# uw-x/AcousticSwarms-Speech

Measured on AMD Instinct MI355X. Metric: TDoA candidates/sec (shift+normalise+spot forward+energies), higher is better.
Workload: dtype f32 via f16x3 split-operand MFMA (fp32 accumulate); 1 GPU; configs[2] scene: 5-speaker reverberant mixture (image sources), 7 mics, T=48000 samples (BASELINE's '3 s @ 16 kHz' sample count; the reference pipeline and this scene generator run at 48 kHz, where it is a 1 s clip -- the reference-native 3 s is extras.T144000), fine-stage (Strict=1) candidate batch of one mixture, FULL spot net 47.27 M params, seeded random weights; internal_batch=256, parallelism=candidate-shard x1

## Files before the change

### acousticswarms-speech_amd/csrc/model_common.h

```cpp
#pragma once
#include <cstdlib>
#include <iterator>
#include <map>
#include <memory>
#include <string>
#include <vector>

#include "asw_common.h"

namespace asw_model {

struct DevBuf {
  float* p = nullptr;
  size_t n = 0;
  DevBuf() = default;
  DevBuf(const DevBuf&) = delete;
  DevBuf& operator=(const DevBuf&) = delete;
  DevBuf(DevBuf&& o) noexcept : p(o.p), n(o.n) { o.p = nullptr; o.n = 0; }
  ~DevBuf() { if (p) (void)hipFree(p); }
  int upload(const std::vector<float>& h) {
    if (p) { (void)hipFree(p); p = nullptr; }
    n = h.size();
    if (hipMalloc(&p, n * sizeof(float)) != hipSuccess) return asw::set_error(ASW_ERR_NOMEM, "hipMalloc(%zu floats)", n);
    ASW_HIP(hipMemcpy(p, h.data(), n * sizeof(float), hipMemcpyHostToDevice));
    return ASW_OK;
  }
};

struct WBuf {
  DevBuf f32;
  uint16_t* hi = nullptr;
  uint16_t* lo = nullptr;
  int32_t shift = 0;
  WBuf() = default;
  WBuf(const WBuf&) = delete;
  WBuf& operator=(const WBuf&) = delete;
  WBuf(WBuf&& o) noexcept : f32(std::move(o.f32)), hi(o.hi), lo(o.lo), shift(o.shift), fhi(o.fhi), flo(o.flo) {
    o.hi = o.lo = o.fhi = o.flo = nullptr;
  }
  ~WBuf() {
    if (hi) (void)hipFree(hi);
    if (lo) (void)hipFree(lo);
    if (fhi) (void)hipFree(fhi);
    if (flo) (void)hipFree(flo);
  }
  int upload_gemm(const std::vector<float>& h, int N, int K) {
    int rc = upload(h);
    if (rc) return rc;
    if (N % 32 == 0 && K % 16 == 0 && (size_t)N * K == h.size()) return upload_frags(h, N, K);
    return ASW_OK;
  }
  int upload(const std::vector<float>& h) {
    int rc = f32.upload(h);
    if (rc) return rc;
    std::vector<uint16_t> vh(h.size()), vl(h.size());
    if ((rc = asw_split_weights_f16(h.data(), h.size(), vh.data(), vl.data(), &shift))) return rc;
    if (hi) { (void)hipFree(hi); hi = nullptr; }
    if (lo) { (void)hipFree(lo); lo = nullptr; }
    if (hipMalloc(&hi, h.size() * 2) != hipSuccess || hipMalloc(&lo, h.size() * 2) != hipSuccess)
      return asw::set_error(ASW_ERR_NOMEM, "hipMalloc(%zu halves)", h.size());
    ASW_HIP(hipMemcpy(hi, vh.data(), h.size() * 2, hipMemcpyHostToDevice));
    ASW_HIP(hipMemcpy(lo, vl.data(), h.size() * 2, hipMemcpyHostToDevice));
    return ASW_OK;
  }
  uint16_t* fhi = nullptr;
  uint16_t* flo = nullptr;
  int upload_frags(const std::vector<float>& h, int N, int K) {
    std::vector<uint16_t> vh(h.size()), vl(h.size());
    int32_t sh = 0;
    int rc = asw_pack_fragments_f16(h.data(), N, K, vh.data(), vl.data(), &sh);
    if (rc) return rc;
    if (sh != shift) return asw::set_error(ASW_ERR_STATE, "fragment pack: inconsistent weight shift");
    if (fhi) { (void)hipFree(fhi); fhi = nullptr; }
    if (flo) { (void)hipFree(flo); flo = nullptr; }
    if (hipMalloc(&fhi, h.size() * 2) != hipSuccess || hipMalloc(&flo, h.size() * 2) != hipSuccess)
      return asw::set_error(ASW_ERR_NOMEM, "hipMalloc(%zu halves)", h.size());
    ASW_HIP(hipMemcpy(fhi, vh.data(), h.size() * 2, hipMemcpyHostToDevice));
    ASW_HIP(hipMemcpy(flo, vl.data(), h.size() * 2, hipMemcpyHostToDevice));
    return ASW_OK;
  }
  void bind(asw_convgemm_args& a, int precision) const {
    a.Wt = f32.p; a.Wt_hi = hi; a.Wt_lo = lo; a.w_shift = shift; a.precision = precision;
    a.Wf_hi = fhi; a.Wf_lo = flo;
  }
};

struct ResLayer { WBuf wt; DevBuf bias, g, b; int dil = 1; };

inline std::vector<float> pack_conv(const std::vector<float>& w, int N, int Cin, int K, const float* in_gate) {
  std::vector<float> o((size_t)N * Cin * K);
  for (int n = 0; n < N; ++n)
    for (int c = 0; c < Cin; ++c)
      for (int k = 0; k < K; ++k)
        o[((size_t)n * K + k) * Cin + c] = w[((size_t)n * Cin + c) * K + k] * (in_gate ? in_gate[c] : 1.f);
  return o;
}


inline int pack_res_layers(const std::map<std::string, std::vector<float>>& raw, const std::string& p, int ch, int K,
                           int n_layers, int dil_factor, std::vector<ResLayer>& out) {
  out.clear();
  out.resize(n_layers);
  int dil = 1;
  for (int j = 0; j < n_layers; ++j) {
    const std::string q = p + ".res.seq." + std::to_string(j);
    int rc;
    {
      const std::vector<float> packed = pack_conv(raw.at(q + ".conv.weight"), ch, ch, K, nullptr);
      if ((rc = out[j].wt.upload(packed))) return rc;
      if (ch % 32 == 0 && (ch * K) % 16 == 0 && (rc = out[j].wt.upload_frags(packed, ch, ch * K))) return rc;
    }
    if ((rc = out[j].bias.upload(raw.at(q + ".conv.bias")))) return rc;
    if ((rc = out[j].g.upload(raw.at(q + ".norm.weight")))) return rc;
    if ((rc = out[j].b.upload(raw.at(q + ".norm.bias")))) return rc;
    out[j].dil = dil;
    dil *= dil_factor;
  }
  return ASW_OK;
}

struct Arena {
  char* base;
  size_t off = 0, cap;
  bool dry;
  Arena(char* b, size_t c, bool d) : base(b), cap(c), dry(d) {}
  template <typename T>
  T* take(size_t n) {
    off = (off + 255) & ~(size_t)255;
    T* p = reinterpret_cast<T*>(base + off);
    off += n * sizeof(T);
    return p;
  }
};


struct GluSrc { const float* raw; const float* mr; const float* gamma; const float* beta; float* side_out = nullptr; };

inline bool glu_on_load_ok(const std::vector<ResLayer>& res, int prec, int ch) {
  static const int max_c = getenv("ASW_GLU_ON_LOAD_MAX_C") ? atoi(getenv("ASW_GLU_ON_LOAD_MAX_C")) : 512;
  return prec >= 1 && (ch == 64 || ch == 128 || ch == 256 || ch == 512) && ch <= max_c && !res.empty() &&
         res[0].dil == 1 && res[0].wt.fhi && res[0].wt.flo;
}

inline bool resstack_ok(const std::vector<ResLayer>& res, int prec, int ch, int K) {
  static const bool off = getenv("ASW_NO_RESSTACK") != nullptr;
  if (off || prec < 1 || ch != 64 || K % 2 == 0 || K < 3 || K > 15) return false;
  for (const ResLayer& r : res)
    if (!r.wt.fhi || !r.wt.flo) return false;
  return true;
}

inline int run_res(const std::vector<ResLayer>& res, int prec, int B, int T, int ch, int K, float* x, float* p, float* q,
            float** final_out, hipStream_t s, const GluSrc* glu = nullptr) {
  const float* in = glu ? glu->raw : x;
  float* outb = p;
  if (resstack_ok(res, prec, ch, K)) {
    static const bool nofuse = getenv("ASW_RESSTACK_NOFUSE") != nullptr;
    size_t j = 0;
    while (j < res.size()) {
      size_t n = 1;
      int halo = 0;
      while (!nofuse && j + n < res.size() && n < 3) {
        const int pad = res[j + n].dil * (K - 1) / 2;
        if (halo + pad > 64) break;
        halo += pad;
        ++n;
      }
      asw_resstack_args a = {};
      a.x = (glu && j == 0) ? nullptr : in;
      a.out = outb;
      a.B = B; a.T = T; a.C = ch; a.taps = K; a.n_layers = (int)n; a.precision = prec; a.ln_eps = 1e-5f;
      for (size_t i = 0; i < n; ++i) {
        const ResLayer& r = res[j + i];
        a.layer[i].Wf_hi = r.wt.fhi; a.layer[i].Wf_lo = r.wt.flo; a.layer[i].w_shift = r.wt.shift;
        a.layer[i].bias = r.bias.p; a.layer[i].ln_gamma = r.g.p; a.layer[i].ln_beta = r.b.p; a.layer[i].dil = r.dil;
      }
      if (glu && j == 0) {
        a.glu_raw = glu->raw; a.glu_mr = glu->mr; a.glu_gamma = glu->gamma; a.glu_beta = glu->beta; a.glu_out = glu->side_out;
      }
      int rc = asw_resstack64_f16x3(&a, s);
      if (rc) return rc;
      in = outb;
      outb = (outb == p) ? q : p;
      j += n;
    }
    *final_out = const_cast<float*>(in);
    return ASW_OK;
  }
  for (size_t j = 0; j < res.size(); ++j) {
    asw_convgemm_args a = {};
    a.A = in; res[j].wt.bind(a, prec); a.bias = res[j].bias.p; a.resid = in;
    if (glu && j == 0) {
      a.glu_raw = glu->raw; a.glu_mr = glu->mr; a.glu_gamma = glu->gamma; a.glu_beta = glu->beta; a.glu_out = glu->side_out;
    }
    a.ln_gamma = res[j].g.p; a.ln_beta = res[j].b.p; a.out = outb;
    a.B = B; a.M_out = T; a.N = ch; a.Cin = ch; a.taps = K; a.stride = 1; a.dil = res[j].dil;
    a.pad = (res[j].dil * (K - 1) + 1) / 2;
    a.a_row_stride = ch; a.a_batch_stride = (int64_t)T * ch; a.a_len = (int64_t)T * ch;
    a.relu = 1; a.ln_eps = 1e-5f;
    int rc = asw_convgemm_f32(&a, s);
    if (rc) return rc;
    in = outb;
    outb = (outb == p) ? q : p;
  }
  *final_out = const_cast<float*>(in);
  return ASW_OK;
}

inline int linear(const float* A, const WBuf& W, int prec, const float* bias, int rows, int N, int K, int relu, const float* resid,
           const float* g, const float* b, float* out, hipStream_t s) {
  asw_convgemm_args a = {};
  a.A = A; W.bind(a, prec); a.bias = bias; a.resid = resid; a.ln_gamma = g; a.ln_beta = b; a.out = out;
  a.B = 1; a.M_out = rows; a.N = N; a.Cin = K; a.taps = 1; a.stride = 1; a.dil = 1; a.pad = 0;
  a.a_row_stride = K; a.a_batch_stride = (int64_t)rows * K; a.a_len = (int64_t)rows * K;
  a.relu = relu; a.ln_eps = 1e-5f;
  if (g && N >= 1024 && N % 256 == 0 && N <= 2048) {
    a.resid = nullptr; a.ln_gamma = nullptr; a.ln_beta = nullptr;
    int rc = asw_convgemm_f32(&a, s);
    if (rc) return rc;
    return asw_add_layernorm(out, resid, g, b, rows, N, 1e-5f, out, s);
  }
  return asw_convgemm_f32(&a, s);
}

inline void pack_conv_transpose(const std::vector<float>& w, const std::vector<float>& b, int Cin, int N, int S,
                                const float* out_gate, std::vector<float>& wt, std::vector<float>& bb) {
  wt.assign((size_t)S * N * Cin, 0.f);
  bb.assign((size_t)S * N, 0.f);
  for (int r = 0; r < S; ++r)
    for (int n = 0; n < N; ++n) {
      bb[(size_t)r * N + n] = out_gate ? b[n] * out_gate[n] : b[n];
      for (int c = 0; c < Cin; ++c) {
        const float v = w[((size_t)c * N + n) * S + r];
        wt[((size_t)r * N + n) * Cin + c] = out_gate ? v * out_gate[n] : v;
      }
    }
}


#define UP(buf, vec) if ((rc = (buf).upload(vec))) return rc

struct TrunkCfg {
  int n_mics, kernel_size, depth, stride_list[8], channels, growth, encoder_channels, encoder_kernel_size,
      encoder_stride, residual_layers, residual_dilation_factor, ffw_dim;
  template <class Cfg>
  static TrunkCfg of(const Cfg& c) {
    TrunkCfg t = {c.n_mics, c.kernel_size, c.depth, {}, c.channels, c.growth, c.encoder_channels,
                  c.encoder_kernel_size, c.encoder_stride, c.residual_layers, c.residual_dilation_factor, c.ffw_dim};
    for (int i = 0; i < 8; ++i) t.stride_list[i] = c.stride_list[i];
    return t;
  }
};

inline int check_trunk_config(const TrunkCfg& c, const char* who, const char* odd) {
  ASW_CHECK_ARG(c.depth >= 1 && c.depth <= 8, "%s: depth %d", who, c.depth);
  ASW_CHECK_ARG(c.n_mics >= 1 && c.n_mics <= 32, "%s: n_mics %d", who, c.n_mics);
  ASW_CHECK_ARG(c.channels % 64 == 0, "%s: channels=%d must be a multiple of 64 for the MFMA tiles", who, c.channels);
  ASW_CHECK_ARG(c.growth >= 1 && c.residual_layers >= 1, "%s: bad config", who);
  ASW_CHECK_ARG(c.kernel_size % 2 == 1, "%s: %s", who, odd);
  ASW_CHECK_ARG(c.encoder_channels % 128 == 0, "%s: encoder_channels must be a multiple of 128", who);
  ASW_CHECK_ARG(c.encoder_stride % 4 == 0 && c.encoder_kernel_size / 2 == c.encoder_stride && c.encoder_kernel_size <= 64,
                "%s: encoder kernel/stride %d/%d unsupported (the reference's trim [9:-8] assumes 33/16)", who,
                c.encoder_kernel_size, c.encoder_stride);
  ASW_CHECK_ARG(c.ffw_dim % 128 == 0, "%s: ffw_dim must be a multiple of 128", who);
  return ASW_OK;
}

struct EncBlock { std::vector<ResLayer> res; DevBuf bias, gn_g, gn_b; };
struct DecBlock { std::vector<ResLayer> res; DevBuf gn_g, gn_b; };
struct GatedConvs { std::vector<WBuf> down_wt, up_wt; std::vector<DevBuf> up_bias; };
struct Tap { const float* p; size_t numel; };
using ParamList = std::vector<std::pair<std::string, size_t>>;

struct TrunkPlan {
  int B, T, Tp, F, RL;
  std::vector<int> Tl;
  float *mean, *stdv, *refn;
  std::vector<float*> X, Pb, Qb, raw_dn, raw_up, st_dn, st_up, mr_dn, mr_up;
  float *Y, *D, *ywave;
};

struct Trunk {
  TrunkCfg tc;
  std::map<std::string, std::vector<float>> raw;
  std::map<std::string, Tap> taps;
  bool finalized = false;
  int device = 0;
  int precision = 0;
  bool fuse_mask = true;

  std::vector<int> enc_cin, enc_cout;
  std::vector<int> dec_cin, dec_cout, dec_stride;
  int stride_product = 1;

  DevBuf pre_w, pre_b;
  std::vector<EncBlock> enc;
  std::vector<DecBlock> dec;
  WBuf byp_wt, mask_wt, dec_wt;
  WBuf byp_wt48;
  DevBuf byp_b, mask_b;
  float out_bias = 0.f;
  int byp_k = 0;

  const std::vector<float>& P(const std::string& k) const { return raw.at(k); }

  int init_shape(const TrunkCfg& c, const char* who) {
    tc = c;
    ASW_HIP(hipGetDevice(&device));
    int cin = c.channels, ch = c.channels;
    for (int i = 0; i < c.depth; ++i) {
      ASW_CHECK_ARG(c.stride_list[i] >= 1, "%s: stride", who);
      enc_cin.push_back(cin);
      enc_cout.push_back(ch);
      stride_product *= c.stride_list[i];
      cin = ch;
      ch *= c.growth;
    }
    dec_cin.assign(enc_cout.rbegin(), enc_cout.rend());
    dec_cout.assign(enc_cin.rbegin(), enc_cin.rend());
    dec_stride.assign(std::make_reverse_iterator(c.stride_list + c.depth), std::make_reverse_iterator(c.stride_list));
    return ASW_OK;
  }
  int check_level_widths(const char* who) const {
    for (int w : enc_cin) ASW_CHECK_ARG(w <= 512 && (w & (w - 1)) == 0, "%s: level width %d must be a power of two <= 512", who, w);
    return ASW_OK;
  }

  ParamList trunk_params() const {
    ParamList v;
    const size_t K = tc.kernel_size;
    v.push_back({"preproc.weight", (size_t)tc.channels * tc.n_mics});
    v.push_back({"preproc.bias", (size_t)tc.channels});
    auto res = [&](const std::string& p, size_t ch) {
      for (int j = 0; j < tc.residual_layers; ++j) {
        const std::string q = p + ".res.seq." + std::to_string(j);
        v.push_back({q + ".conv.weight", ch * ch * K});
        v.push_back({q + ".conv.bias", ch});
        v.push_back({q + ".norm.weight", ch});
        v.push_back({q + ".norm.bias", ch});
      }
    };
    for (int i = 0; i < tc.depth; ++i) {
      const std::string p = "encoder.module_list." + std::to_string(i);
      const size_t ci = enc_cin[i], co = enc_cout[i];
      res(p, ci);
      v.push_back({p + ".conv1.weight", 2 * co * ci * K});
      v.push_back({p + ".conv1.bias", 2 * co});
      v.push_back({p + ".norm1.weight", 2 * co});
      v.push_back({p + ".norm1.bias", 2 * co});
    }
    for (int i = 0; i < tc.depth; ++i) {
      const std::string p = "decoder.module_list." + std::to_string(i);
      const size_t ci = dec_cin[i], co = dec_cout[i], s = dec_stride[i];
      v.push_back({p + ".upsample.conv.weight", ci * 2 * co * s});
      v.push_back({p + ".upsample.conv.bias", 2 * co});
      v.push_back({p + ".norm1.weight", 2 * co});
      v.push_back({p + ".norm1.bias", 2 * co});
      res(p, co);
    }
    const size_t E = tc.encoder_channels, EK = tc.encoder_kernel_size;
    v.push_back({"reference_bypass.weight", E * EK});
    v.push_back({"reference_bypass.bias", E});
    v.push_back({"mask_encoder.weight", E * tc.channels * EK});
    v.push_back({"mask_encoder.bias", E});
    v.push_back({"output_decoder.weight", E * EK});
    v.push_back({"output_decoder.bias", 1});
    return v;
  }

  int finalize_trunk(const char* who, const ParamList& want) {
    {
      int dev = -1;
      ASW_HIP(hipGetDevice(&dev));
      if (dev != device)
        return asw::set_error(ASW_ERR_STATE, "%s: model was created on HIP device %d, current device is %d", who, device, dev);
    }
    for (const auto& kv : want) {
      auto it = raw.find(kv.first);
      if (it == raw.end()) return asw::set_error(ASW_ERR_STATE, "state dict is missing key %s", kv.first.c_str());
      if (it->second.size() != kv.second)
        return asw::set_error(ASW_ERR_ARG, "%s: %zu elements, expected %zu", kv.first.c_str(), it->second.size(), kv.second);
    }
    if (raw.size() != want.size())
      return asw::set_error(ASW_ERR_ARG, "state dict has %zu unexpected keys", raw.size() - want.size());
    int rc;
    const int K = tc.kernel_size, RL = tc.residual_layers, RD = tc.residual_dilation_factor;
    UP(pre_w, P("preproc.weight"));
    UP(pre_b, P("preproc.bias"));
    enc.clear(); enc.resize(tc.depth);
    dec.clear(); dec.resize(tc.depth);
    for (int i = 0; i < tc.depth; ++i) {
      const std::string p = "encoder.module_list." + std::to_string(i);
      if ((rc = pack_res_layers(raw, p, enc_cin[i], K, RL, RD, enc[i].res))) return rc;
      UP(enc[i].bias, P(p + ".conv1.bias"));
      UP(enc[i].gn_g, P(p + ".norm1.weight"));
      UP(enc[i].gn_b, P(p + ".norm1.bias"));
    }
    for (int i = 0; i < tc.depth; ++i) {
      const std::string p = "decoder.module_list." + std::to_string(i);
      if ((rc = pack_res_layers(raw, p, dec_cout[i], K, RL, RD, dec[i].res))) return rc;
      UP(dec[i].gn_g, P(p + ".norm1.weight"));
      UP(dec[i].gn_b, P(p + ".norm1.bias"));
    }
    const int E = tc.encoder_channels, EK = tc.encoder_kernel_size;
    byp_k = ((EK + 31) / 32) * 32;
    {
      const std::vector<float>& w = P("reference_bypass.weight");
      std::vector<float> wt((size_t)E * byp_k, 0.f);
      for (int n = 0; n < E; ++n)
        for (int k = 0; k < EK; ++k) wt[(size_t)n * byp_k + k] = w[(size_t)n * EK + k];
      UP(byp_wt, wt);
      UP(byp_b, P("reference_bypass.bias"));
      if (E % 32 == 0 && EK <= 48) {
        std::vector<float> w48((size_t)E * 48, 0.f);
        for (int n = 0; n < E; ++n)
          for (int k = 0; k < EK; ++k) w48[(size_t)n * 48 + k] = w[(size_t)n * EK + k];
        if ((rc = byp_wt48.upload_gemm(w48, E, 48))) return rc;
      }
    }
    if ((rc = mask_wt.upload_gemm(pack_conv(P("mask_encoder.weight"), E, tc.channels, EK, nullptr), E, tc.channels * EK))) return rc;
    UP(mask_b, P("mask_encoder.bias"));
    {
      const std::vector<float>& w = P("output_decoder.weight");
      std::vector<float> wt((size_t)64 * E, 0.f);
      for (int j = 0; j < EK; ++j)
        for (int e = 0; e < E; ++e) wt[(size_t)j * E + e] = w[(size_t)e * EK + j];
      if ((rc = dec_wt.upload_gemm(wt, 64, E))) return rc;
      out_bias = P("output_decoder.bias")[0];
    }
    return ASW_OK;
  }

  template <class Gate>
  int pack_gated(GatedConvs& o, Gate gate) const {
    const int K = tc.kernel_size;
    int rc;
    o.down_wt.clear(); o.down_wt.resize(tc.depth);
    o.up_wt.clear(); o.up_wt.resize(tc.depth);
    o.up_bias.clear(); o.up_bias.resize(tc.depth);
    for (int i = 0; i < tc.depth; ++i) {
      const std::string p = "encoder.module_list." + std::to_string(i);
      const std::vector<float> g = gate(p);
      const int n = 2 * enc_cout[i], ci = enc_cin[i];
      if ((rc = o.down_wt[i].upload_gemm(pack_conv(P(p + ".conv1.weight"), n, ci, K, g.empty() ? nullptr : g.data()), n, ci * K)))
        return rc;
    }
    for (int j = 0; j < tc.depth; ++j) {
      const std::string p = "decoder.module_list." + std::to_string(j);
      const std::vector<float> g = gate(p);
      const int ci = dec_cin[j], co2 = 2 * dec_cout[j], s = dec_stride[j];
      std::vector<float> wt, bb;
      pack_conv_transpose(P(p + ".upsample.conv.weight"), P(p + ".upsample.conv.bias"), ci, co2, s,
                          g.empty() ? nullptr : g.data(), wt, bb);
      if ((rc = o.up_wt[j].upload_gemm(wt, s * co2, ci))) return rc;
      UP(o.up_bias[j], bb);
    }
    return ASW_OK;
  }

  bool fused_mask_path() const {
    return fuse_mask && precision >= 1 && tc.encoder_channels % 256 == 0 && tc.channels % 32 == 0 &&
           tc.encoder_kernel_size <= 48 && tc.encoder_stride % 4 == 0 && byp_wt48.fhi && dec_wt.fhi && mask_wt.fhi;
  }
  void layout_levels(int B, int T, Arena& a, TrunkPlan& pl) const {
    const int depth = tc.depth, EK = tc.encoder_kernel_size, ES = tc.encoder_stride;
    pl.B = B; pl.T = T;
    pl.Tp = ((T - 1) / stride_product + 1) * stride_product;
    pl.F = (pl.Tp + 2 * (EK / 2) - EK) / ES + 1;
    pl.RL = ((EK / 2 + pl.Tp + byp_k + 64) + 3) & ~3;
    pl.Tl.assign(depth + 1, pl.Tp);
    for (int i = 0; i < depth; ++i) pl.Tl[i + 1] = pl.Tl[i] / tc.stride_list[i];
    pl.mean = a.take<float>(B);
    pl.stdv = a.take<float>(B);
    pl.refn = a.take<float>((size_t)B * pl.RL);
    pl.X.resize(depth + 1); pl.Pb.resize(depth); pl.Qb.resize(depth);
    pl.raw_dn.resize(depth); pl.raw_up.resize(depth); pl.st_dn.resize(depth); pl.st_up.resize(depth);
    pl.mr_up.resize(depth); pl.mr_dn.resize(depth);
    for (int i = 0; i <= depth; ++i) {
      const int ch = i == 0 ? tc.channels : enc_cout[i - 1];
      pl.X[i] = a.take<float>((size_t)B * pl.Tl[i] * ch);
    }
    for (int i = 0; i < depth; ++i) {
      const size_t n = (size_t)B * pl.Tl[i] * enc_cin[i];
      pl.Pb[i] = a.take<float>(n);
      pl.Qb[i] = a.take<float>(n);
      pl.raw_dn[i] = a.take<float>((size_t)B * pl.Tl[i + 1] * 2 * enc_cout[i]);
      pl.st_dn[i] = a.take<float>((size_t)B * 4 * asw_convgemm_stats_tiles(pl.Tl[i + 1], 2 * enc_cout[i]));
      pl.mr_dn[i] = a.take<float>((size_t)B * 4);
    }
    for (int j = 0; j < depth; ++j) {
      const int lvl = depth - j;
      const int s = dec_stride[j], co2 = 2 * dec_cout[j];
      pl.raw_up[j] = a.take<float>((size_t)B * pl.Tl[lvl] * s * co2);
      pl.st_up[j] = a.take<float>((size_t)B * 4 * asw_convgemm_stats_tiles(pl.Tl[lvl], s * co2));
      pl.mr_up[j] = a.take<float>((size_t)B * 4);
    }
  }
  void layout_mask(Arena& a, TrunkPlan& pl) const {
    const int E = tc.encoder_channels;
    const bool fused = fused_mask_path();
    pl.Y = fused ? nullptr : a.take<float>((size_t)pl.B * pl.F * E);
    pl.D = a.take<float>((size_t)(fused ? E / 256 : 1) * pl.B * pl.F * 64);
    pl.ywave = a.take<float>((size_t)pl.B * pl.T);
  }

  int encode(TrunkPlan& pl, const GatedConvs& g, hipStream_t s) {
    const int B = pl.B, K = tc.kernel_size;
    taps.clear();
    taps["preproc"] = {pl.X[0], (size_t)B * pl.Tl[0] * tc.channels};
    int rc;
    GluSrc src = {};
    bool glu = false;
    for (int i = 0; i < tc.depth; ++i) {
      float* r = nullptr;
      if ((rc = run_res(enc[i].res, precision, B, pl.Tl[i], enc_cin[i], K, pl.X[i], pl.Pb[i], pl.Qb[i], &r, s,
                        glu ? &src : nullptr)))
        return rc;
      asw_convgemm_args a = {};
      a.A = r; g.down_wt[i].bind(a, precision); a.bias = enc[i].bias.p; a.out = pl.raw_dn[i]; a.stats = pl.st_dn[i];
      a.B = B; a.M_out = pl.Tl[i + 1]; a.N = 2 * enc_cout[i]; a.Cin = enc_cin[i]; a.taps = K;
      a.stride = tc.stride_list[i]; a.dil = 1; a.pad = K / 2;
      a.a_row_stride = a.Cin; a.a_batch_stride = (int64_t)pl.Tl[i] * a.Cin; a.a_len = a.a_batch_stride;
      a.chan_mod = a.N;
      if ((rc = asw_convgemm_f32(&a, s))) return rc;
      glu = fuse_mask && i + 1 < tc.depth && glu_on_load_ok(enc[i + 1].res, precision, enc_cout[i]);
      const int tiles = asw_convgemm_stats_tiles(a.M_out, a.N);
      if (glu) {
        if ((rc = asw_gn_finalize(pl.st_dn[i], tiles, B, pl.Tl[i + 1], enc_cout[i], 1e-5f, pl.mr_dn[i], s))) return rc;
        src = {pl.raw_dn[i], pl.mr_dn[i], enc[i].gn_g.p, enc[i].gn_b.p, pl.X[i + 1]};
      } else if ((rc = asw_gn_glu(pl.raw_dn[i], pl.st_dn[i], tiles, enc[i].gn_g.p, enc[i].gn_b.p, B, pl.Tl[i + 1],
                                  enc_cout[i], 1e-5f, pl.X[i + 1], s))) {
        return rc;
      }
      taps["enc" + std::to_string(i)] = {pl.X[i + 1], (size_t)B * pl.Tl[i + 1] * enc_cout[i]};
    }
    return ASW_OK;
  }

  int decode(TrunkPlan& pl, const GatedConvs& g, const float*& x, hipStream_t s) {
    const int B = pl.B, K = tc.kernel_size;
    int rc;
    for (int j = 0; j < tc.depth; ++j) {
      const int lvl = tc.depth - j, ci = dec_cin[j], co = dec_cout[j], st = dec_stride[j];
      asw_convgemm_args a = {};
      a.A = x; a.A2 = pl.X[lvl]; g.up_wt[j].bind(a, precision); a.bias = g.up_bias[j].p; a.out = pl.raw_up[j];
      a.stats = pl.st_up[j];
      a.B = B; a.M_out = pl.Tl[lvl]; a.N = st * 2 * co; a.Cin = ci; a.taps = 1; a.stride = 1; a.dil = 1; a.pad = 0;
      a.a_row_stride = ci; a.a_batch_stride = (int64_t)pl.Tl[lvl] * ci; a.a_len = a.a_batch_stride;
      a.chan_mod = 2 * co;
      if ((rc = asw_convgemm_f32(&a, s))) return rc;
      const int To = pl.Tl[lvl] * st;
      const int tiles = asw_convgemm_stats_tiles(a.M_out, a.N);
      float* gb = pl.Qb[lvl - 1];
      float* r = nullptr;
      if (fuse_mask && glu_on_load_ok(dec[j].res, precision, co)) {
        if ((rc = asw_gn_finalize(pl.st_up[j], tiles, B, To, co, 1e-5f, pl.mr_up[j], s))) return rc;
        const GluSrc src = {pl.raw_up[j], pl.mr_up[j], dec[j].gn_g.p, dec[j].gn_b.p, co > 64 ? gb : nullptr};
        if ((rc = run_res(dec[j].res, precision, B, To, co, K, gb, pl.Pb[lvl - 1], gb, &r, s, &src))) return rc;
      } else {
        if ((rc = asw_gn_glu(pl.raw_up[j], pl.st_up[j], tiles, dec[j].gn_g.p, dec[j].gn_b.p, B, To, co, 1e-5f, gb, s)))
          return rc;
        if ((rc = run_res(dec[j].res, precision, B, To, co, K, gb, pl.Pb[lvl - 1], gb, &r, s))) return rc;
      }
      x = r;
      taps["dec" + std::to_string(j)] = {x, (size_t)B * To * co};
    }
    return ASW_OK;
  }

  int mask_path(TrunkPlan& pl, const float* x, const float* mean, const float* stdv, float* out_wave, hipStream_t s) {
    const int B = pl.B, C = tc.channels, E = tc.encoder_channels, EK = tc.encoder_kernel_size, ES = tc.encoder_stride;
    int rc;
    asw_convgemm_args me = {};
    me.A = x; mask_wt.bind(me, precision); me.bias = mask_b.p;
    me.B = B; me.M_out = pl.F; me.N = E; me.Cin = C; me.taps = EK; me.stride = ES; me.dil = 1; me.pad = EK / 2;
    me.a_row_stride = C; me.a_batch_stride = (int64_t)pl.Tp * C; me.a_len = me.a_batch_stride;
    if (fused_mask_path()) {
      asw_maskpath_args f = {};
      f.enc = me;
      f.ref = pl.refn; f.ref_batch_stride = pl.RL; f.ref_len = pl.RL; f.ref_hop = ES;
      f.byp_k = 48; f.byp_taps = EK; f.byp_shift = byp_wt48.shift; f.byp_hi = byp_wt48.fhi; f.byp_lo = byp_wt48.flo;
      f.byp_bias = byp_b.p;
      f.dec_hi = dec_wt.fhi; f.dec_lo = dec_wt.flo; f.dec_shift = dec_wt.shift; f.dec_taps = EK;
      f.taps = pl.D;
      if ((rc = asw_mask_path_f16x3(&f, s))) return rc;
      return asw_overlap_add_parts(pl.D, E / 256, B, pl.F, 64, EK, EK / 2, pl.T, 9, 8, out_bias, mean, stdv, out_wave, s);
    }
    {
      asw_convgemm_args a = {};
      a.A = pl.refn; byp_wt.bind(a, precision); a.bias = byp_b.p; a.out = pl.Y;
      a.B = B; a.M_out = pl.F; a.N = E; a.Cin = byp_k; a.taps = 1; a.stride = 1; a.dil = 1; a.pad = 0;
      a.a_row_stride = ES; a.a_batch_stride = pl.RL; a.a_len = pl.RL; a.relu = 1;
      if ((rc = asw_convgemm_f32(&a, s))) return rc;
    }
    me.mul = pl.Y; me.out = pl.Y; me.relu = 1;
    if ((rc = asw_convgemm_f32(&me, s))) return rc;
    taps["latent"] = {pl.Y, (size_t)B * pl.F * E};
    {
      asw_convgemm_args a = {};
      a.A = pl.Y; dec_wt.bind(a, precision); a.out = pl.D;
      a.B = B; a.M_out = pl.F; a.N = 64; a.Cin = E; a.taps = 1; a.stride = 1; a.dil = 1; a.pad = 0;
      a.a_row_stride = E; a.a_batch_stride = (int64_t)pl.F * E; a.a_len = a.a_batch_stride;
      if ((rc = asw_convgemm_f32(&a, s))) return rc;
    }
    return asw_overlap_add_unnorm(pl.D, B, pl.F, 64, EK, EK / 2, pl.T, 9, 8, out_bias, mean, stdv, out_wave, s);
  }
};

inline int check_ready(const Trunk* m, const char* fin) {
  if (!m) return asw::set_error(ASW_ERR_ARG, "null model handle");
  if (!m->finalized) return asw::set_error(ASW_ERR_STATE, "%s() has not been called", fin);
  int dev = -1;
  ASW_HIP(hipGetDevice(&dev));
  if (dev != m->device)
    return asw::set_error(ASW_ERR_STATE, "model lives on HIP device %d but the current device is %d", m->device, dev);
  return ASW_OK;
}

inline int set_precision(Trunk* m, const char* who, int precision) {
  ASW_CHECK_ARG(m && (precision >= 0 && precision <= 2), "%s: 0 (f32), 1 (f16x3) or 2 (single-pass f16)", who);
  m->precision = precision;
  return ASW_OK;
}

inline int set_param(Trunk* m, const char* who, const char* key, const float* host_data, size_t numel) {
  ASW_CHECK_ARG(m && key && host_data, "%s: null pointer", who);
  m->raw[key].assign(host_data, host_data + numel);
  m->finalized = false;
  return ASW_OK;
}

inline int get_tap(const Trunk* m, const char* who, const char* name, float* dst, size_t capacity, size_t* numel,
                   void* stream) {
  ASW_CHECK_ARG(m && name && numel, "%s: null pointer", who);
  auto it = m->taps.find(name);
  if (it == m->taps.end()) return asw::set_error(ASW_ERR_ARG, "%s: no activation named %s", who, name);
  *numel = it->second.numel;
  if (dst) {
    ASW_CHECK_ARG(capacity >= it->second.numel, "%s: buffer too small", who);
    ASW_HIP(hipMemcpyAsync(dst, it->second.p, it->second.numel * sizeof(float), hipMemcpyDeviceToDevice,
                           asw::as_stream(stream)));
  }
  return ASW_OK;
}

}
```

### acousticswarms-speech_amd/csrc/prep_kernels.hip

```cpp
#include "asw_common.h"

namespace {

constexpr int MAX_MICS = 32;

__device__ __forceinline__ float quant16(float x) {
  return rintf(x * 32768.0f) * (1.0f / 32768.0f);
}

__device__ __forceinline__ double block_sum(double v, double* red) {
#pragma unroll
  for (int o = 32; o > 0; o >>= 1) v += __shfl_xor(v, o, 64);
  const int lane = threadIdx.x & 63, wid = threadIdx.x >> 6, nw = blockDim.x >> 6;
  __syncthreads();
  if (lane == 0) red[wid] = v;
  __syncthreads();
  double s = 0.0;
  for (int i = 0; i < nw; ++i) s += red[i];
  return s;
}

__global__ __launch_bounds__(1024) void shift_stats_kernel(const float* __restrict__ mixes, int M, int T,
                                                           const int32_t* __restrict__ offsets,
                                                           const int32_t* __restrict__ mix_index, int circular,
                                                           float* __restrict__ mean_out,
                                                           float* __restrict__ std_out) {
  __shared__ int off[MAX_MICS];
  __shared__ double red[16];
  const int n = blockIdx.x;
  const float* __restrict__ mix = mixes + (mix_index ? (long)mix_index[n] * M * T : 0);
  if (threadIdx.x < M) {
    int o = threadIdx.x == 0 ? 0 : offsets[(long)n * (M - 1) + threadIdx.x - 1];
    if (circular) { o %= T; if (o < 0) o += T; }
    off[threadIdx.x] = o;
  }
  __syncthreads();
  const float inv_m = 1.0f / (float)M;
  auto ref_at = [&](int t) -> float {
    float s = 0.f;
    for (int m = 0; m < M; ++m) {
      int i = t + off[m];
      float x;
      if (circular) { if (i >= T) i -= T; x = mix[(long)m * T + i]; }
      else x = (i >= 0 && i < T) ? mix[(long)m * T + i] : 0.f;
      s += quant16(x);
    }
    return s * inv_m;
  };
  double acc = 0.0;
  for (int t = threadIdx.x; t < T; t += blockDim.x) acc += (double)ref_at(t);
  const double mean = block_sum(acc, red) / (double)T;
  acc = 0.0;
  for (int t = threadIdx.x; t < T; t += blockDim.x) {
    const double d = (double)ref_at(t) - mean;
    acc += d * d;
  }
  const double var = block_sum(acc, red) / (double)(T - 1);
  if (threadIdx.x == 0) {
    mean_out[n] = (float)mean;
    std_out[n] = (float)sqrt(var);
  }
}

template <bool SHIFTED>
__global__ __launch_bounds__(256) void preproc_kernel(const float* __restrict__ srcs, int M, int T, int T_pad,
                                                      const int32_t* __restrict__ offsets,
                                                      const int32_t* __restrict__ mix_index, int circular,
                                                      const float* __restrict__ mean, const float* __restrict__ stdv,
                                                      const float* __restrict__ w, const float* __restrict__ bias,
                                                      int C, float* __restrict__ x0, float* __restrict__ refn,
                                                      long refn_stride, int rows_per_block) {
  __shared__ int off[MAX_MICS];
  __shared__ float vs[64 * MAX_MICS];
  __shared__ float ws[128 * MAX_MICS];
  const int n = blockIdx.y;
  const float* __restrict__ src = srcs + ((SHIFTED && mix_index) ? (long)mix_index[n] * M * T : 0);
  for (int i = threadIdx.x; i < C * M; i += blockDim.x) ws[i] = w[i];
  const int c4n = C >> 2;
  if (threadIdx.x < M) {
    int o = 0;
    if (SHIFTED && threadIdx.x > 0) {
      o = offsets[(long)n * (M - 1) + threadIdx.x - 1];
      if (circular) { o %= T; if (o < 0) o += T; }
    }
    off[threadIdx.x] = o;
  }
  __syncthreads();
  const int pad = T_pad - T;
  const float mu = SHIFTED ? mean[n] : 0.f;
  const float sg = SHIFTED ? stdv[n] : 1.f;
  const int row0 = blockIdx.x * rows_per_block;
  for (int it = threadIdx.x; it < rows_per_block * M; it += blockDim.x) {
    const int m = it / rows_per_block, r = it - m * rows_per_block;
    const int tp = row0 + r;
    float x = 0.f;
    if (tp >= pad && tp < T_pad) {
      const int t = tp - pad;
      if (SHIFTED) {
        int i = t + off[m];
        if (circular) { if (i >= T) i -= T; x = src[(long)m * T + i]; }
        else x = (i >= 0 && i < T) ? src[(long)m * T + i] : 0.f;
        x = (quant16(x) - mu) / sg;
      } else {
        x = src[((long)n * M + m) * T + t];
      }
    }
    vs[r * M + m] = x;
  }
  __syncthreads();
  const int items = rows_per_block * c4n;
  for (int it = threadIdx.x; it < items; it += blockDim.x) {
    const int r = it / c4n, c4 = it - r * c4n;
    const int tp = row0 + r;
    if (tp >= T_pad) break;
    const int c = c4 * 4;
    float4 o = *reinterpret_cast<const float4*>(bias + c);
    if (tp >= pad) {
      for (int m = 0; m < M; ++m) {
        const float x = vs[r * M + m];
        o.x = fmaf(ws[(c + 0) * M + m], x, o.x);
        o.y = fmaf(ws[(c + 1) * M + m], x, o.y);
        o.z = fmaf(ws[(c + 2) * M + m], x, o.z);
        o.w = fmaf(ws[(c + 3) * M + m], x, o.w);
      }
    }
    *reinterpret_cast<float4*>(x0 + ((long)n * T_pad + tp) * C + c) = o;
    if (c4 == 0) refn[(long)n * refn_stride + tp] = vs[r * M];
  }
}

}

extern "C" int asw_shift_stats(const float* mix, int M, int T, const int32_t* offsets, int N, int circular,
                               float* mean, float* std, void* stream) {
  return asw_shift_stats_multi(mix, M, T, offsets, nullptr, N, circular, mean, std, stream);
}

extern "C" int asw_shift_stats_multi(const float* mix, int M, int T, const int32_t* offsets, const int32_t* mix_index, int N,
                                     int circular, float* mean, float* std, void* stream) {
  ASW_CHECK_ARG(mix && offsets && mean && std, "shift_stats: null pointer");
  ASW_CHECK_ARG(M >= 1 && M <= MAX_MICS && T >= 2, "shift_stats: M=%d T=%d unsupported", M, T);
  if (N == 0) return ASW_OK;
  asw::ProfScope prof(asw::as_stream(stream), "shift_stats", 0.0, (double)M * T * 4 + (double)N * 8);
  hipLaunchKernelGGL(shift_stats_kernel, dim3(N), dim3(1024), 0, asw::as_stream(stream), mix, M, T, offsets, mix_index,
                     circular, mean, std);
  ASW_LAUNCH_CHECK();
  return ASW_OK;
}

extern "C" int asw_shift_norm_preproc(const float* mix, int M, int T, int T_pad, const int32_t* offsets, int N,
                                      int circular, const float* mean, const float* std, const float* w,
                                      const float* b, int C, float* x0, float* refn, long refn_stride,
                                      void* stream) {
  return asw_shift_norm_preproc_multi(mix, M, T, T_pad, offsets, nullptr, N, circular, mean, std, w, b, C, x0, refn,
                                      refn_stride, stream);
}

extern "C" int asw_shift_norm_preproc_multi(const float* mix, int M, int T, int T_pad, const int32_t* offsets,
                                            const int32_t* mix_index, int N, int circular, const float* mean,
                                            const float* std, const float* w, const float* b, int C, float* x0, float* refn,
                                            long refn_stride, void* stream) {
  ASW_CHECK_ARG(refn_stride >= T_pad, "shift_norm_preproc: refn_stride < T_pad");
  ASW_CHECK_ARG(mix && offsets && mean && std && w && b && x0 && refn, "shift_norm_preproc: null pointer");
  ASW_CHECK_ARG(M >= 1 && M <= MAX_MICS && T >= 1 && T_pad >= T && C % 4 == 0 && C > 0 && C <= 128,
                "shift_norm_preproc: bad shape M=%d T=%d T_pad=%d C=%d (C <= 128)", M, T, T_pad, C);
  if (N == 0) return ASW_OK;
  const int rows = 64;
  dim3 grid(asw::cdiv(T_pad, rows), N);
  asw::ProfScope prof(asw::as_stream(stream), "preproc", 0.0, (double)M * T * 4 + (double)N * T_pad * (C + 1) * 4);
  hipLaunchKernelGGL(preproc_kernel<true>, grid, dim3(256), 0, asw::as_stream(stream), mix, M, T, T_pad, offsets, mix_index,
                     circular, mean, std, w, b, C, x0, refn, refn_stride, rows);
  ASW_LAUNCH_CHECK();
  return ASW_OK;
}

extern "C" int asw_pad_preproc(const float* x, int B, int M, int t, int T_pad, const float* w, const float* b,
                               int C, float* x0, float* refn, long refn_stride, void* stream) {
  ASW_CHECK_ARG(refn_stride >= T_pad, "pad_preproc: refn_stride < T_pad");
  ASW_CHECK_ARG(x && w && b && x0 && refn, "pad_preproc: null pointer");
  ASW_CHECK_ARG(M >= 1 && M <= MAX_MICS && t >= 1 && T_pad >= t && C % 4 == 0 && C > 0 && C <= 128,
                "pad_preproc: bad shape M=%d t=%d T_pad=%d C=%d (C <= 128)", M, t, T_pad, C);
  if (B == 0) return ASW_OK;
  const int rows = 64;
  dim3 grid(asw::cdiv(T_pad, rows), B);
  hipLaunchKernelGGL(preproc_kernel<false>, grid, dim3(256), 0, asw::as_stream(stream), x, M, t, T_pad,
                     (const int32_t*)nullptr, (const int32_t*)nullptr, 1, (const float*)nullptr, (const float*)nullptr, w, b, C, x0, refn,
                     refn_stride, rows);
  ASW_LAUNCH_CHECK();
  return ASW_OK;
}
```

### acousticswarms-speech_amd/csrc/resstack.hip

```cpp
#include <type_traits>

#include "asw_common.h"
#include "f16x3_tile.h"

namespace {
using namespace asw_mfma;

constexpr int C = 64;
constexpr int MAXL = 3;

struct LayerDev {
  const half8* Wh;
  const half8* Wl;
  const float* bias;
  const float* gamma;
  const float* beta;
  int dil, pad;
  int halo;
  int nfrag;
  float scale;
};

#ifdef ASW_PHASE_TIMING
__device__ unsigned long long g_rs_cycles[6] = {0, 0, 0, 0, 0, 0};
#define RS_MARK(var) const unsigned long long var = __builtin_readcyclecounter()
#else
#define RS_MARK(var)
#endif

struct KArgs {
  const float* x;
  float* out;
  const float* glu_raw;
  const float* glu_mr;
  const float* glu_gamma;
  const float* glu_beta;
  float* glu_out;
  int B, T, taps, ntile, BM, img_rows;
  float eps;
  LayerDev L[MAXL];
};

template <int NL, int NW, int TM, int PH, bool POLY, bool GLU, int NTERM, int QD>
__global__ __launch_bounds__(64 * NW) __attribute__((amdgpu_waves_per_eu(TM >= 4 ? 1 : 2)))
void resstack64_kernel(const KArgs p) {
  static_assert(!POLY || NL == 1, "polyphase row sets: single layers only");
  static_assert(QD == 2 || QD == 4, "weight prefetch depth in k-steps");
  constexpr int NTHR = 64 * NW, SROWS = NTHR / 16;
  constexpr int R0 = 32 * NW * TM;
  constexpr int BMJ = R0 / PH;
  static_assert(BMJ % 32 == 0, "a row fragment must stay inside one phase");

  extern __shared__ __align__(16) char smem[];
  char* img = smem;
  float* tab = reinterpret_cast<float*>(smem + (size_t)p.img_rows * RS);

  const int tid = threadIdx.x, lane = tid & 63, wid = tid >> 6;
  int idx;
  if (!xcd_tile_run(p.B * p.ntile, idx)) return;
  const int b = idx / p.ntile, tile = idx - b * p.ntile;
  const int T = p.T, taps = p.taps;
  const int dil0 = p.L[0].dil, pad0 = p.L[0].pad;
  const int n_pb = POLY ? (dil0 + PH - 1) / PH : 1;
  const int jb = POLY ? tile / n_pb : 0, pb = POLY ? tile - jb * n_pb : 0;
  const int m0 = tile * p.BM;
  const int RJ = BMJ + taps - 1;
  const int R_img = POLY ? PH * RJ : R0 + 2 * pad0;

  RS_MARK(t_start);
  for (int i = tid; i < NL * 3 * 16; i += NTHR) {
    const int li = i / 48, w = (i - li * 48) / 16, c4 = i & 15;
    const float* src = w == 0 ? p.L[li].bias : w == 1 ? p.L[li].gamma : p.L[li].beta;
    reinterpret_cast<float4*>(tab)[i] = *reinterpret_cast<const float4*>(src + c4 * 4);
  }
  {
    const __amdgpu_buffer_rsrc_t rX = GLU ? act_rsrc(p.glu_raw + (long)b * T * 2 * C, (long)T * 2 * C)
                                          : act_rsrc(p.x + (long)b * T * C, (long)T * C);
    const int srow = tid >> 4, sc4 = tid & 15;
    GluCoef gc;
    if (GLU) {
      gc.stats(p.glu_mr, b);
      gc.affine(p.glu_gamma, p.glu_beta, C, sc4 * 4);
    }
    constexpr int SU = GLU ? 9 : 18;
    for (int r0 = 0; r0 < R_img; r0 += SROWS * SU) {
      float4 buf[SU];
      float4 gate[GLU ? SU : 1];
      bool okr[GLU ? SU : 1];
#pragma unroll
      for (int u = 0; u < SU; ++u) {
        const int row = r0 + u * SROWS + srow;
        int g;
        bool ok = row < R_img;
        if (!POLY) {
          g = m0 - p.L[0].halo - pad0 + row;
        } else {
          const int ph = pb * PH + row / RJ;
          const int jj = jb * BMJ + row % RJ - (taps - 1) / 2;
          g = dil0 * jj + ph;
          ok = ok && ph < dil0 && jj >= 0;
        }
        ok = ok && g >= 0 && g < T;
        if (GLU) {
          buf[u] = act_load4(rX, (long)g * 2 * C + sc4 * 4, ok);
          gate[u] = act_load4(rX, (long)g * 2 * C + C + sc4 * 4, ok);
          okr[u] = ok;
        } else {
          buf[u] = act_load4(rX, (long)g * C + sc4 * 4, ok);
        }
      }
      if (GLU) {
#pragma unroll
        for (int u = 0; u < SU; ++u) {
          const float4 o = gn_glu4(buf[u], gate[u], gc, okr[u]);
          buf[u] = o;
          if (p.glu_out && okr[u]) {
            const int g = m0 - p.L[0].halo - pad0 + r0 + u * SROWS + srow;
            if (g >= m0 && g < m0 + p.BM)
              *reinterpret_cast<float4*>(p.glu_out + ((long)b * T + g) * C + sc4 * 4) = o;
          }
        }
      }
#pragma unroll
      for (int u = 0; u < SU; ++u) {
        const int row = r0 + u * SROWS + srow;
        if (row < R_img) {
          half4 hi, lo;
          split4t<NTERM>(buf[u], hi, lo);
          *reinterpret_cast<half4*>(img + row * RS + IMG_HI + sc4 * 8) = hi;
          *reinterpret_cast<half4*>(img + row * RS + IMG_LO + sc4 * 8) = lo;
        }
      }
    }
  }
  __syncthreads();
  RS_MARK(t_staged);
#ifdef ASW_PHASE_TIMING
  unsigned long long t_marks[2 * MAXL + 1];
  t_marks[0] = t_staged;
#endif

  const int h = lane >> 5;
  floatx16 acc[TM][2];
  auto layer = [&](auto lic) {
    constexpr int li = decltype(lic)::value;
    constexpr bool last = li == NL - 1;
    const LayerDev& Ld = p.L[li];
    const int tapstep = (POLY ? 1 : Ld.dil) * RS;
    const int nf = Ld.nfrag - wid * TM;
#pragma unroll
    for (int i = 0; i < TM; ++i)
#pragma unroll
      for (int cb = 0; cb < 2; ++cb)
#pragma unroll
        for (int r = 0; r < 16; ++r) acc[i][cb][r] = 0.f;
    auto img_row = [&](int trow) { return POLY ? (trow / BMJ) * RJ + trow % BMJ : trow; };
    auto run = [&](auto nfc) {
      constexpr int NF = decltype(nfc)::value;
      int xb[NF];
      floatx16 a[NF][2];
#pragma unroll
      for (int i = 0; i < NF; ++i) {
        xb[i] = (img_row((wid * TM + i) * 32) + (lane & 31)) * RS + h * 16;
        a[i][0] = acc[i][0];
        a[i][1] = acc[i][1];
      }
      kloop<NF, 2, QD, NTERM>(
          a, taps, [&](int tap, int i) __attribute__((always_inline)) { return img + xb[i] + tap * tapstep; }, Ld.Wh, Ld.Wl,
          [](int kg, int cb) __attribute__((always_inline)) { return (long)kg * 2 + cb; }, lane);
#pragma unroll
      for (int i = 0; i < NF; ++i) { acc[i][0] = a[i][0]; acc[i][1] = a[i][1]; }
    };
    if (nf >= TM) run(std::integral_constant<int, TM>{});
    else if constexpr (TM > 1) {
      if (nf == 1) run(std::integral_constant<int, 1>{});
      if constexpr (TM > 2) {
        if (nf == 2) run(std::integral_constant<int, 2>{});
        if (nf == 3) run(std::integral_constant<int, 3>{});
      }
    }
#ifdef ASW_PHASE_TIMING
    {
      float sink = acc[0][0][0];
      asm volatile("" ::"v"(sink));
      t_marks[2 * li + 1] = __builtin_readcyclecounter();
    }
#endif
    const float* tb = tab + li * 192;
    const int cpad = POLY ? (taps - 1) / 2 : Ld.pad;
#pragma unroll
    for (int i = 0; i < TM; ++i) {
      if (i < nf) {
        const int trow = (wid * TM + i) * 32 + (lane & 31);
        const char* rrow = img + (img_row(trow) + cpad) * RS;
        float s = 0.f;
#pragma unroll
        for (int cb = 0; cb < 2; ++cb)
#pragma unroll
          for (int q = 0; q < 4; ++q) {
            const int c0 = cb * 32 + q * 8 + h * 4;
            const float4 bi = *reinterpret_cast<const float4*>(tb + c0);
            const half4 rh = *reinterpret_cast<const half4*>(rrow + IMG_HI + c0 * 2);
            const half4 rl = *reinterpret_cast<const half4*>(rrow + IMG_LO + c0 * 2);
            const float bv[4] = {bi.x, bi.y, bi.z, bi.w};
#pragma unroll
            for (int j = 0; j < 4; ++j) {
              float v = fmaxf(acc[i][cb][q * 4 + j] * Ld.scale + bv[j], 0.f);
              v += (float)rh[j] + (float)rl[j];
              acc[i][cb][q * 4 + j] = v;
              s += v;
            }
          }
        s += __shfl_xor(s, 32, 64);
        const float mean = s * (1.0f / C);
        float d = 0.f;
#pragma unroll
        for (int cb = 0; cb < 2; ++cb)
#pragma unroll
          for (int r = 0; r < 16; ++r) { const float cx = acc[i][cb][r] - mean; d += cx * cx; }
        d += __shfl_xor(d, 32, 64);
        const float rstd = 1.0f / sqrtf(d * (1.0f / C) + p.eps);
#pragma unroll
        for (int cb = 0; cb < 2; ++cb)
#pragma unroll
          for (int q = 0; q < 4; ++q) {
            const int c0 = cb * 32 + q * 8 + h * 4;
            const float4 g4 = *reinterpret_cast<const float4*>(tb + 64 + c0);
            const float4 b4 = *reinterpret_cast<const float4*>(tb + 128 + c0);
            const float gv[4] = {g4.x, g4.y, g4.z, g4.w}, be[4] = {b4.x, b4.y, b4.z, b4.w};
#pragma unroll
            for (int j = 0; j < 4; ++j) acc[i][cb][q * 4 + j] = (acc[i][cb][q * 4 + j] - mean) * rstd * gv[j] + be[j];
          }
      }
    }
    if constexpr (!last) {
      __syncthreads();
#pragma unroll
      for (int i = 0; i < TM; ++i) {
        if (i < nf) {
          const int trow = (wid * TM + i) * 32 + (lane & 31);
          const int t = m0 - Ld.halo + trow;
          const bool inside = t >= 0 && t < T;
          char* wrow = img + trow * RS;
#pragma unroll
          for (int cb = 0; cb < 2; ++cb)
#pragma unroll
            for (int q = 0; q < 4; ++q) {
              const int c0 = cb * 32 + q * 8 + h * 4;
              float4 v = make_float4(acc[i][cb][q * 4 + 0], acc[i][cb][q * 4 + 1], acc[i][cb][q * 4 + 2], acc[i][cb][q * 4 + 3]);
              if (!inside) v = make_float4(0.f, 0.f, 0.f, 0.f);
              half4 hi, lo;
              split4t<NTERM>(v, hi, lo);
              *reinterpret_cast<half4*>(wrow + IMG_HI + c0 * 2) = hi;
              *reinterpret_cast<half4*>(wrow + IMG_LO + c0 * 2) = lo;
            }
        }
      }
      __syncthreads();
    } else {
      float* __restrict__ ob = p.out + (long)b * T * C;
#pragma unroll
      for (int i = 0; i < TM; ++i) {
        if (i < nf) {
          const int trow = (wid * TM + i) * 32 + (lane & 31);
          int t;
          bool ok;
          if (!POLY) {
            t = m0 + trow;
            ok = trow < p.BM && t < T;
          } else {
            const int ph = pb * PH + trow / BMJ;
            t = dil0 * (jb * BMJ + trow % BMJ) + ph;
            ok = ph < dil0 && t < T;
          }
          if (ok) {
            float* orow = ob + (long)t * C;
#pragma unroll
            for (int cb = 0; cb < 2; ++cb)
#pragma unroll
              for (int q = 0; q < 4; ++q) {
                const int c0 = cb * 32 + q * 8 + h * 4;
                *reinterpret_cast<float4*>(orow + c0) =
                    make_float4(acc[i][cb][q * 4 + 0], acc[i][cb][q * 4 + 1], acc[i][cb][q * 4 + 2], acc[i][cb][q * 4 + 3]);
              }
          }
        }
      }
    }
  };
  layer(std::integral_constant<int, 0>{});
#ifdef ASW_PHASE_TIMING
  t_marks[2] = __builtin_readcyclecounter();
#endif
  if constexpr (NL > 1) layer(std::integral_constant<int, 1>{});
  if constexpr (NL > 2) layer(std::integral_constant<int, 2>{});
#ifdef ASW_PHASE_TIMING
  if (threadIdx.x == 0 && NL <= 2) {
    const unsigned long long t_end = __builtin_readcyclecounter();
    atomicAdd(&g_rs_cycles[0], t_staged - t_start);
    atomicAdd(&g_rs_cycles[1], t_marks[1] - t_marks[0]);
    if (NL == 1) {
      atomicAdd(&g_rs_cycles[4], t_end - t_marks[1]);
    } else {
      atomicAdd(&g_rs_cycles[2], t_marks[2] - t_marks[1]);
      atomicAdd(&g_rs_cycles[3], t_marks[3] - t_marks[2]);
      atomicAdd(&g_rs_cycles[4], t_end - t_marks[3]);
    }
    atomicAdd(&g_rs_cycles[5], 1ull);
  }
#endif
}

template <int NL, int NW, int TM, int PH, bool POLY, bool GLU, int QD>
int launch_stack(const KArgs& k, int precision, size_t smem, double flops, const char* tag, hipStream_t s) {
  char nm[128], detail[48] = "";
  snprintf(nm, sizeof nm, "resstack64<%s,%dx%d%s%s>", tag, NW, TM, POLY ? (PH == 1 ? ",poly1" : PH == 2 ? ",poly2" : ",poly4") : "",
           GLU ? ",glu" : "");
  if (asw::prof_detail()) snprintf(detail, sizeof detail, "[B%d M%d d%d]", k.B, k.T, k.L[0].dil);
  return asw::launch_pair<resstack64_kernel<NL, NW, TM, PH, POLY, GLU, 1, QD>, resstack64_kernel<NL, NW, TM, PH, POLY, GLU, 3, QD>>(
      precision, dim3(xcd_grid_run(k.B * k.ntile)), dim3(64 * NW), smem, 160 * 1024, nm, detail, flops,
      (double)k.B * k.T * C * 4 * (GLU ? 3 : 2), s, k);
}

template <int NW, int TM>
int dispatch(const asw_resstack_args& a, KArgs& k, bool glu, double flops, hipStream_t s) {
  constexpr int R0 = 32 * NW * TM;
  const int dil0 = k.L[0].dil;
  const int rpp = a.T / dil0;
  if (a.n_layers == 1 && dil0 >= 7 && rpp >= 48 && !glu) {
    const int PH = rpp >= R0 - 32 ? 1 : rpp >= R0 / 2 - 32 ? 2 : 4;
    const int BMJ = R0 / PH;
    k.BM = R0;
    k.L[0].nfrag = NW * TM;
    k.ntile = asw::cdiv(asw::cdiv(a.T, dil0), BMJ) * asw::cdiv(dil0, PH);
    k.img_rows = PH * (BMJ + a.taps - 1);
    const size_t smem = (size_t)k.img_rows * RS + 3 * 64 * sizeof(float);
    switch (PH) {
      case 1: return launch_stack<1, NW, TM, 1, true, false, 4>(k, a.precision, smem, flops, "1", s);
      case 2: return launch_stack<1, NW, TM, 2, true, false, 4>(k, a.precision, smem, flops, "1", s);
      default: return launch_stack<1, NW, TM, 4, true, false, 4>(k, a.precision, smem, flops, "1", s);
    }
  }
  k.BM = R0 - 2 * k.L[0].halo;
  ASW_CHECK_ARG(k.BM >= R0 / 2, "resstack: the later layers' halo (%d rows per side) leaves %d of %d rows; fuse fewer layers",
                k.L[0].halo, k.BM, R0);
  k.ntile = asw::cdiv(a.T, k.BM);
  int rows = 0;
  for (int i = 0; i < a.n_layers; ++i) {
    k.L[i].nfrag = asw::cdiv(k.BM + 2 * k.L[i].halo, 32);
    const int r = 32 * k.L[i].nfrag + 2 * k.L[i].pad;
    rows = r > rows ? r : rows;
  }
  k.img_rows = rows;
  const size_t smem = (size_t)rows * RS + (size_t)a.n_layers * 3 * 64 * sizeof(float);
  ASW_CHECK_ARG(smem <= 160 * 1024, "resstack: image of %d rows exceeds LDS (dilation %d x %d taps too wide for a contiguous tile)",
                rows, dil0, a.taps);
  switch (a.n_layers) {
    case 1: return glu ? launch_stack<1, NW, TM, 1, false, true, 4>(k, a.precision, smem, flops, "1", s)
                       : launch_stack<1, NW, TM, 1, false, false, 4>(k, a.precision, smem, flops, "1", s);
    case 2: return glu ? launch_stack<2, NW, TM, 1, false, true, 4>(k, a.precision, smem, flops, "2", s)
                       : launch_stack<2, NW, TM, 1, false, false, 4>(k, a.precision, smem, flops, "2", s);
    default: return glu ? launch_stack<3, NW, TM, 1, false, true, 4>(k, a.precision, smem, flops, "3", s)
                        : launch_stack<3, NW, TM, 1, false, false, 4>(k, a.precision, smem, flops, "3", s);
  }
}

}

#ifdef ASW_PHASE_TIMING
extern "C" int asw_debug_resstack_cycles(unsigned long long* out6, int reset) {
  ASW_HIP(hipMemcpyFromSymbol(out6, HIP_SYMBOL(g_rs_cycles), 6 * sizeof(unsigned long long)));
  if (reset) {
    const unsigned long long z[6] = {0, 0, 0, 0, 0, 0};
    ASW_HIP(hipMemcpyToSymbol(HIP_SYMBOL(g_rs_cycles), z, sizeof z));
  }
  return ASW_OK;
}
#endif

extern "C" int asw_resstack64_f16x3(const asw_resstack_args* args, void* stream) {
  ASW_CHECK_ARG(args != nullptr, "resstack: null args");
  const asw_resstack_args& a = *args;
  hipStream_t s = asw::as_stream(stream);
  ASW_CHECK_ARG(a.C == C, "resstack: C=%d (64 only)", a.C);
  ASW_CHECK_ARG(a.n_layers >= 1 && a.n_layers <= MAXL, "resstack: 1..%d layers", MAXL);
  ASW_CHECK_ARG(a.taps >= 3 && a.taps <= 15 && a.taps % 2 == 1, "resstack: taps=%d (odd, 3..15)", a.taps);
  ASW_CHECK_ARG(a.precision == 1 || a.precision == 2, "resstack: precision 1 (f16x3) or 2 (single-pass f16)");
  ASW_CHECK_ARG(a.B > 0 && a.B <= (1 << 20) && a.T > 0 && (int64_t)a.T * 2 * C < ((int64_t)1 << 29), "resstack: bad B / T");
  ASW_CHECK_ARG(a.out && (a.x || a.glu_raw), "resstack: null tensor");
  const bool glu = a.glu_raw != nullptr;
  if (glu) ASW_CHECK_ARG(a.glu_mr && a.glu_gamma && a.glu_beta, "resstack: GroupNorm + GLU on load needs the statistics / affine arrays");
  KArgs k = {};
  k.x = a.x; k.out = a.out; k.glu_raw = a.glu_raw; k.glu_mr = a.glu_mr; k.glu_gamma = a.glu_gamma; k.glu_beta = a.glu_beta;
  k.glu_out = glu ? a.glu_out : nullptr;
  k.B = a.B; k.T = a.T; k.taps = a.taps; k.eps = a.ln_eps;
  int halo = 0;
  for (int i = a.n_layers - 1; i >= 0; --i) {
    const asw_reslayer_desc& d = a.layer[i];
    ASW_CHECK_ARG(d.Wf_hi && d.Wf_lo && d.bias && d.ln_gamma && d.ln_beta && d.dil >= 1, "resstack: layer %d incomplete", i);
    LayerDev& L = k.L[i];
    L.Wh = reinterpret_cast<const half8*>(d.Wf_hi); L.Wl = reinterpret_cast<const half8*>(d.Wf_lo);
    L.bias = d.bias; L.gamma = d.ln_gamma; L.beta = d.ln_beta;
    L.dil = d.dil; L.pad = d.dil * (a.taps - 1) / 2; L.halo = halo;
    L.scale = ldexpf(1.0f, -d.w_shift);
    halo += L.pad;
  }
  const double flops = 2.0 * a.B * (double)a.T * C * C * a.taps * a.n_layers;
  return dispatch<4, 2>(a, k, glu, flops, s);
}
```

### acousticswarms-speech_amd/csrc/spot_model.hip

```cpp
#include <map>
#include <memory>
#include <string>
#include <vector>

#include "model_common.h"

using namespace asw_model;

namespace {

struct TfLayer { WBuf w_in, w_out, w1, w2; DevBuf b_in, b_out, b1, b2, n1g, n1b, n2g, n2b; };
struct GateSet : GatedConvs { uint64_t stamp = 0; };

}

struct asw_spot : Trunk {
  asw_spot_config cfg;
  int batch = 32;
  uint64_t clock = 0;
  std::vector<TfLayer> tf;
  std::map<std::pair<float, float>, std::unique_ptr<GateSet>> gates;

  char* ws[2] = {nullptr, nullptr};
  size_t ws_bytes[2] = {0, 0};
  int lanes = 1;
  hipStream_t side = nullptr;
  hipEvent_t ev_fork = nullptr, ev_join = nullptr;

  ~asw_spot() {
    for (char* w : ws) if (w) (void)hipFree(w);
    if (side) (void)hipStreamDestroy(side);
    if (ev_fork) (void)hipEventDestroy(ev_fork);
    if (ev_join) (void)hipEventDestroy(ev_join);
  }
};

namespace {

ParamList expected_params(const asw_spot* m) {
  const asw_spot_config& c = m->cfg;
  ParamList v = m->trunk_params();
  for (int i = 0; i < c.depth; ++i) {
    const std::string p = "encoder.module_list." + std::to_string(i);
    v.push_back({p + ".embed1.weight", (size_t)m->enc_cin[i] * 2});
    v.push_back({p + ".embed1.bias", (size_t)m->enc_cin[i]});
  }
  for (int i = 0; i < c.depth; ++i) {
    const std::string p = "decoder.module_list." + std::to_string(i);
    v.push_back({p + ".embed1.weight", (size_t)2 * m->dec_cout[i] * 2});
    v.push_back({p + ".embed1.bias", (size_t)2 * m->dec_cout[i]});
  }
  const size_t d = m->enc_cout.back(), f = c.ffw_dim;
  for (int l = 0; l < c.num_transformer_layers; ++l) {
    const std::string p = "bottleneck.transf.layers." + std::to_string(l);
    v.push_back({p + ".self_attn.in_proj_weight", 3 * d * d});
    v.push_back({p + ".self_attn.in_proj_bias", 3 * d});
    v.push_back({p + ".self_attn.out_proj.weight", d * d});
    v.push_back({p + ".self_attn.out_proj.bias", d});
    v.push_back({p + ".linear1.weight", f * d});
    v.push_back({p + ".linear1.bias", f});
    v.push_back({p + ".linear2.weight", d * f});
    v.push_back({p + ".linear2.bias", d});
    v.push_back({p + ".norm1.weight", d});
    v.push_back({p + ".norm1.bias", d});
    v.push_back({p + ".norm2.weight", d});
    v.push_back({p + ".norm2.bias", d});
  }
  return v;
}

std::vector<float> gate_of(const std::vector<float>& w, const std::vector<float>& b, float w0, float w1) {
  std::vector<float> g(b.size());
  for (size_t c = 0; c < b.size(); ++c) g[c] = w[2 * c] * w0 + w[2 * c + 1] * w1 + b[c];
  return g;
}

int get_gates(asw_spot* m, float w0, float w1, GateSet** out) {
  auto key = std::make_pair(w0, w1);
  auto it = m->gates.find(key);
  if (it != m->gates.end()) { it->second->stamp = ++m->clock; *out = it->second.get(); return ASW_OK; }
  if (m->gates.size() >= 8) {
    auto lru = m->gates.begin();
    for (auto g = m->gates.begin(); g != m->gates.end(); ++g)
      if (g->second->stamp < lru->second->stamp) lru = g;
    m->gates.erase(lru);
  }
  std::unique_ptr<GateSet> gs(new GateSet());
  gs->stamp = ++m->clock;
  int rc = m->pack_gated(*gs, [&](const std::string& p) {
    return gate_of(m->P(p + ".embed1.weight"), m->P(p + ".embed1.bias"), w0, w1);
  });
  if (rc) return rc;
  *out = gs.get();
  m->gates[key] = std::move(gs);
  return ASW_OK;
}

struct Plan : TrunkPlan {
  float *qkv, *ctx, *x1, *ff, *ha, *hb;
  double* escr;
};

void layout(const asw_spot* m, int B, int T, Arena& a, Plan& pl) {
  m->layout_levels(B, T, a, pl);
  const size_t L = pl.Tl[m->cfg.depth], d = m->enc_cout.back(), rows = (size_t)B * L;
  pl.qkv = a.take<float>(rows * 3 * d);
  pl.ctx = a.take<float>(rows * d);
  pl.x1 = a.take<float>(rows * d);
  pl.ff = a.take<float>(rows * m->cfg.ffw_dim);
  pl.ha = a.take<float>(rows * d);
  pl.hb = a.take<float>(rows * d);
  m->layout_mask(a, pl);
  pl.escr = a.take<double>((size_t)B * (T + 1));
}

int ensure_ws(asw_spot* m, int B, int T, Plan& pl, int lane = 0) {
  Arena dry(nullptr, 0, true);
  layout(m, B, T, dry, pl);
  const size_t need = dry.off + 4096;
  if (need > m->ws_bytes[lane]) {
    size_t want = need;
    if (B < m->batch) {
      Plan full;
      Arena dry_full(nullptr, 0, true);
      layout(m, m->batch, T, dry_full, full);
      want = dry_full.off + 4096;
    }
    if (m->ws[lane]) { ASW_HIP(hipDeviceSynchronize()); (void)hipFree(m->ws[lane]); m->ws[lane] = nullptr; m->ws_bytes[lane] = 0; }
    if (hipMalloc(&m->ws[lane], want) != hipSuccess) {
      (void)hipGetLastError();
      want = need;
      if (hipMalloc(&m->ws[lane], want) != hipSuccess)
        return asw::set_error(ASW_ERR_NOMEM, "workspace of %.1f MiB for batch %d, T=%d", need / 1048576.0, B, T);
    }
    m->ws_bytes[lane] = want;
  }
  Arena real(m->ws[lane], m->ws_bytes[lane], false);
  layout(m, B, T, real, pl);
  return ASW_OK;
}

int run_network(asw_spot* m, Plan& pl, GateSet* gs, const float* mean, const float* stdv, float* out_wave,
                hipStream_t s) {
  const asw_spot_config& c = m->cfg;
  int rc;
  if ((rc = m->encode(pl, *gs, s))) return rc;
  const int L = pl.Tl[c.depth], d = m->enc_cout.back(), rows = pl.B * L;
  const float* h = pl.X[c.depth];
  for (int l = 0; l < c.num_transformer_layers; ++l) {
    TfLayer& t = m->tf[l];
    float* hout = (l % 2 == 0) ? pl.ha : pl.hb;
    if ((rc = linear(h, t.w_in, m->precision, t.b_in.p, rows, 3 * d, d, 0, nullptr, nullptr, nullptr, pl.qkv, s))) return rc;
    if ((rc = asw_attention_prec(pl.qkv, pl.B, L, d, c.num_head, m->precision, pl.ctx, s))) return rc;
    if ((rc = linear(pl.ctx, t.w_out, m->precision, t.b_out.p, rows, d, d, 0, h, t.n1g.p, t.n1b.p, pl.x1, s))) return rc;
    if ((rc = linear(pl.x1, t.w1, m->precision, t.b1.p, rows, c.ffw_dim, d, 1, nullptr, nullptr, nullptr, pl.ff, s))) return rc;
    if ((rc = linear(pl.ff, t.w2, m->precision, t.b2.p, rows, d, c.ffw_dim, 0, pl.x1, t.n2g.p, t.n2b.p, hout, s))) return rc;
    h = hout;
  }
  m->taps["bottleneck"] = {h, (size_t)rows * d};
  if ((rc = m->decode(pl, *gs, h, s))) return rc;
  return m->mask_path(pl, h, mean, stdv, out_wave, s);
}

}

extern "C" int asw_spot_create(const asw_spot_config* cfg, asw_spot** out) {
  ASW_CHECK_ARG(cfg && out, "spot_create: null pointer");
  const asw_spot_config& c = *cfg;
  const TrunkCfg tc = TrunkCfg::of(c);
  int rc = check_trunk_config(tc, "spot_create", "kernel_size must be odd");
  if (rc) return rc;
  ASW_CHECK_ARG(c.num_transformer_layers >= 0, "spot_create: bad config");
  std::unique_ptr<asw_spot> m(new asw_spot());
  m->cfg = c;
  if ((rc = m->init_shape(tc, "spot_create"))) return rc;
  const int d = m->enc_cout.back();
  ASW_CHECK_ARG(d <= 1024 && (d & (d - 1)) == 0, "spot_create: bottleneck width %d must be a power of two <= 1024", d);
  ASW_CHECK_ARG(d % c.num_head == 0 && (d / c.num_head) % 16 == 0 && d / c.num_head <= 128,
                "spot_create: head_dim %d unsupported", d / (c.num_head ? c.num_head : 1));
  if ((rc = m->check_level_widths("spot_create"))) return rc;
  *out = m.release();
  return ASW_OK;
}

extern "C" void asw_spot_destroy(asw_spot* m) { delete m; }

extern "C" int asw_spot_set_precision(asw_spot* m, int precision) { return set_precision(m, "set_precision", precision); }

extern "C" int asw_spot_set_batch(asw_spot* m, int batch) {
  ASW_CHECK_ARG(m && batch >= 1 && batch <= 4096, "set_batch: bad argument");
  m->batch = batch;
  return ASW_OK;
}

extern "C" int asw_spot_set_param(asw_spot* m, const char* key, const float* host_data, size_t numel) {
  return set_param(m, "set_param", key, host_data, numel);
}

extern "C" int asw_spot_finalize(asw_spot* m) {
  ASW_CHECK_ARG(m, "finalize: null handle");
  const asw_spot_config& c = m->cfg;
  int rc = m->finalize_trunk("finalize", expected_params(m));
  if (rc) return rc;
  m->tf.clear(); m->tf.resize(c.num_transformer_layers);
  for (int l = 0; l < c.num_transformer_layers; ++l) {
    const std::string p = "bottleneck.transf.layers." + std::to_string(l);
    TfLayer& t = m->tf[l];
    {
      const int dm = m->enc_cout.back(), ff = c.ffw_dim;
      if ((rc = t.w_in.upload_gemm(m->P(p + ".self_attn.in_proj_weight"), 3 * dm, dm))) return rc;
      if ((rc = t.w_out.upload_gemm(m->P(p + ".self_attn.out_proj.weight"), dm, dm))) return rc;
      if ((rc = t.w1.upload_gemm(m->P(p + ".linear1.weight"), ff, dm))) return rc;
      if ((rc = t.w2.upload_gemm(m->P(p + ".linear2.weight"), dm, ff))) return rc;
    }
    UP(t.b_in, m->P(p + ".self_attn.in_proj_bias"));
    UP(t.b_out, m->P(p + ".self_attn.out_proj.bias"));
    UP(t.b1, m->P(p + ".linear1.bias"));
    UP(t.b2, m->P(p + ".linear2.bias"));
    UP(t.n1g, m->P(p + ".norm1.weight")); UP(t.n1b, m->P(p + ".norm1.bias"));
    UP(t.n2g, m->P(p + ".norm2.weight")); UP(t.n2b, m->P(p + ".norm2.bias"));
  }
  m->gates.clear();
  m->finalized = true;
  return ASW_OK;
}

extern "C" int asw_spot_shift_and_sep(asw_spot* m, const float* mix, int M, int T, const int32_t* offsets, int N,
                                      int strict, int circular, float* out_wave, double* out_energy,
                                      int energy_window, void* stream) {
  return asw_spot_shift_and_sep_multi(m, mix, 1, M, T, offsets, nullptr, N, strict, circular, out_wave, out_energy,
                                      energy_window, stream);
}

extern "C" int asw_spot_shift_and_sep_multi(asw_spot* m, const float* mix, int K, int M, int T, const int32_t* offsets,
                                            const int32_t* mix_index, int N, int strict, int circular, float* out_wave,
                                            double* out_energy, int energy_window, void* stream) {
  int rc = check_ready(m, "asw_spot_finalize");
  ASW_CHECK_ARG(K >= 1 && (K == 1 || mix_index != nullptr), "shift_and_sep: K=%d mixtures need a mix_index array", K);
  if (rc) return rc;
  ASW_CHECK_ARG(N >= 0, "shift_and_sep: N=%d", N);
  if (N == 0) return ASW_OK;
  ASW_CHECK_ARG(mix && offsets, "shift_and_sep: null pointer");
  ASW_CHECK_ARG(M == m->cfg.n_mics, "shift_and_sep: mixture has %d channels, model expects %d", M, m->cfg.n_mics);
  ASW_CHECK_ARG(T >= 2, "shift_and_sep: T=%d", T);
  ASW_CHECK_ARG(out_energy == nullptr || energy_window > 0, "shift_and_sep: energy_window");
  hipStream_t s = asw::as_stream(stream);
  GateSet* gs = nullptr;
  if ((rc = get_gates(m, strict == 1 ? 1.f : 0.f, strict == 1 ? 0.f : 1.f, &gs))) return rc;
  const int Bmax = N < m->batch ? N : m->batch;
  const int n_batches = (N + Bmax - 1) / Bmax;
  const int lanes = (m->lanes == 2 && n_batches >= 2) ? 2 : 1;
  Plan pl[2];
  for (int l = 0; l < lanes; ++l)
    if ((rc = ensure_ws(m, Bmax, T, pl[l], l))) return rc;
  hipStream_t st[2] = {s, s};
  if (lanes == 2) {
    if (!m->side) {
      ASW_HIP(hipStreamCreateWithFlags(&m->side, hipStreamNonBlocking));
      ASW_HIP(hipEventCreateWithFlags(&m->ev_fork, hipEventDisableTiming));
      ASW_HIP(hipEventCreateWithFlags(&m->ev_join, hipEventDisableTiming));
    }
    st[1] = m->side;
    ASW_HIP(hipEventRecord(m->ev_fork, s));
    ASW_HIP(hipStreamWaitEvent(m->side, m->ev_fork, 0));
  }
  const int C = m->cfg.channels, pad_l = m->cfg.encoder_kernel_size / 2;
  auto batches = [&]() -> int {
    int k = 0;
    for (int i0 = 0; i0 < N; i0 += Bmax, ++k) {
      const int B = N - i0 < Bmax ? N - i0 : Bmax;
      Plan& p = pl[k % lanes];
      hipStream_t q = st[k % lanes];
      p.B = B;
      const int32_t* off = offsets + (size_t)i0 * (M - 1);
      const int32_t* mi = mix_index ? mix_index + i0 : nullptr;
      ASW_HIP(hipMemsetAsync(p.refn, 0, (size_t)B * p.RL * sizeof(float), q));
      int r;
      if ((r = asw_shift_stats_multi(mix, M, T, off, mi, B, circular, p.mean, p.stdv, q))) return r;
      if ((r = asw_shift_norm_preproc_multi(mix, M, T, p.Tp, off, mi, B, circular, p.mean, p.stdv, m->pre_w.p, m->pre_b.p, C,
                                            p.X[0], p.refn + pad_l, p.RL, q)))
        return r;
      float* y = out_wave ? out_wave + (size_t)i0 * T : p.ywave;
      if ((r = run_network(m, p, gs, p.mean, p.stdv, y, q))) return r;
      if (out_energy && (r = asw_energies(y, B, T, energy_window, p.escr, out_energy + (size_t)i0 * 2, q))) return r;
    }
    return ASW_OK;
  };
  rc = batches();
  if (lanes == 2) {
    if (hipEventRecord(m->ev_join, m->side) != hipSuccess || hipStreamWaitEvent(s, m->ev_join, 0) != hipSuccess) {
      (void)hipStreamSynchronize(m->side);
      if (!rc) rc = asw::set_error(ASW_ERR_HIP, "shift_and_sep: joining the side lane failed");
    }
  }
  return rc;
}

extern "C" int asw_spot_set_lanes(asw_spot* m, int lanes) {
  ASW_CHECK_ARG(m && (lanes == 1 || lanes == 2), "set_lanes: 1 or 2");
  m->lanes = lanes;
  return ASW_OK;
}

extern "C" int asw_spot_forward(asw_spot* m, const float* mix_norm, int B, int M, int t,
                                const float* window_embedding_host, float* out, void* stream) {
  int rc = check_ready(m, "asw_spot_finalize");
  if (rc) return rc;
  ASW_CHECK_ARG(B >= 0, "forward: B=%d", B);
  if (B == 0) return ASW_OK;
  ASW_CHECK_ARG(mix_norm && window_embedding_host && out, "forward: null pointer");
  ASW_CHECK_ARG(M == m->cfg.n_mics && t >= 1, "forward: bad shape");
  hipStream_t s = asw::as_stream(stream);
  GateSet* gs = nullptr;
  if ((rc = get_gates(m, window_embedding_host[0], window_embedding_host[1], &gs))) return rc;
  const int Bmax = B < m->batch ? B : m->batch;
  Plan pl;
  if ((rc = ensure_ws(m, Bmax, t, pl))) return rc;
  const int C = m->cfg.channels, pad_l = m->cfg.encoder_kernel_size / 2;
  for (int i0 = 0; i0 < B; i0 += Bmax) {
    const int b = B - i0 < Bmax ? B - i0 : Bmax;
    pl.B = b;
    ASW_HIP(hipMemsetAsync(pl.refn, 0, (size_t)b * pl.RL * sizeof(float), s));
    if ((rc = asw_pad_preproc(mix_norm + (size_t)i0 * M * t, b, M, t, pl.Tp, m->pre_w.p, m->pre_b.p, C, pl.X[0],
                              pl.refn + pad_l, pl.RL, s)))
      return rc;
    if ((rc = run_network(m, pl, gs, nullptr, nullptr, out + (size_t)i0 * t, s))) return rc;
  }
  return ASW_OK;
}

extern "C" int asw_spot_set_fused_mask(asw_spot* m, int on) {
  ASW_CHECK_ARG(m, "set_fused_mask: null model handle");
  m->fuse_mask = on != 0;
  return ASW_OK;
}

extern "C" int asw_spot_get_tap(asw_spot* m, const char* name, float* dst, size_t capacity, size_t* numel,
                                void* stream) {
  return get_tap(m, "get_tap", name, dst, capacity, numel, stream);
}
```

### acousticswarms-speech_amd/native.py

```python
import ctypes
import os
import subprocess
import sys
from ctypes import (POINTER, Structure, c_char_p, c_double, c_float, c_int, c_int32, c_int64,
                    c_long, c_size_t, c_void_p)

_HERE = os.path.dirname(os.path.abspath(__file__))
LIB_PATH = os.environ.get("ASW_LIB_PATH") or os.path.join(_HERE, "libasw_hip.so")
CSRC = os.path.join(_HERE, "csrc")
SOURCES = ["asw_common.cpp", "convgemm.hip", "resstack.hip", "downconv.hip", "prep_kernels.hip", "misc_kernels.hip", "attention_mfma.hip", "srp_kernels.hip",
           "pruner_kernels.hip", "geometry_kernels.hip",
           "search_host.cpp", "sep_kernels.hip", "spot_model.hip", "sep_model.hip"]
HEADERS = ["asw_common.h", "model_common.h", "mfma_util.h", "f16x3_tile.h"]
EXTRA_FLAGS = {"geometry_kernels.hip": ["-ffp-contract=off"]}
OPS_PATH = os.path.join(_HERE, "libasw_torch_ops.so")
OPS_SOURCE = "torch_ops.cpp"


def build(force: bool = False, verbose: bool = False) -> str:
    from concurrent.futures import ThreadPoolExecutor
    hdrs = [os.path.join(CSRC, h) for h in HEADERS] + [os.path.join(os.path.dirname(_HERE), "include", "asw_hip.h")]
    hdr_time = max(os.path.getmtime(h) for h in hdrs)
    objdir = os.path.join(_HERE, "build")
    os.makedirs(objdir, exist_ok=True)
    jobs, objs = [], []
    for src in SOURCES:
        sp = os.path.join(CSRC, src)
        op = os.path.join(objdir, os.path.splitext(src)[0] + ".o")
        objs.append(op)
        if force or not os.path.exists(op) or os.path.getmtime(op) < max(os.path.getmtime(sp), hdr_time):
            jobs.append(["hipcc", "-O3", "--offload-arch=gfx950", "-std=c++17", "-fPIC"] + EXTRA_FLAGS.get(src, [])
                        + ["-c", sp, "-o", op])
    if not jobs and os.path.exists(LIB_PATH) and all(os.path.getmtime(LIB_PATH) >= os.path.getmtime(o) for o in objs):
        return LIB_PATH

    def run(cmd):
        if verbose:
            print(" ".join(cmd), file=sys.stderr)
        subprocess.run(cmd, check=True)
    with ThreadPoolExecutor(max_workers=min(6, max(1, len(jobs)))) as ex:
        list(ex.map(run, jobs))
    run(["hipcc", "--offload-arch=gfx950", "-fPIC", "-shared", "-o", LIB_PATH] + objs)
    return LIB_PATH


def build_torch_ops(force: bool = False, verbose: bool = False) -> str:
    import torch
    src = os.path.join(CSRC, OPS_SOURCE)
    hdr = os.path.join(os.path.dirname(_HERE), "include", "asw_hip.h")
    if not force and os.path.exists(OPS_PATH) and os.path.getmtime(OPS_PATH) >= max(
            os.path.getmtime(src), os.path.getmtime(hdr), os.path.getmtime(LIB_PATH)):
        return OPS_PATH
    ti = os.path.dirname(torch.__file__)
    cmd = ["hipcc", "-O2", "-std=c++17", "-fPIC", "-shared", "-D__HIP_PLATFORM_AMD__=1", "-DUSE_ROCM=1",
           f"-D_GLIBCXX_USE_CXX11_ABI={int(torch._C._GLIBCXX_USE_CXX11_ABI)}", "-w",
           f"-I{ti}/include", f"-I{ti}/include/torch/csrc/api/include", "-I/opt/rocm/include", src, "-o", OPS_PATH,
           f"-L{_HERE}", "-lasw_hip", f"-L{ti}/lib", "-ltorch", "-ltorch_cpu", "-lc10", "-lc10_hip", "-ltorch_hip",
           "-Wl,-rpath,$ORIGIN", f"-Wl,-rpath,{ti}/lib"]
    if verbose:
        print(" ".join(cmd), file=sys.stderr)
    subprocess.run(cmd, check=True)
    return OPS_PATH


class SpotConfigC(Structure):
    _fields_ = [("n_mics", c_int32), ("kernel_size", c_int32), ("depth", c_int32),
                ("stride_list", c_int32 * 8), ("channels", c_int32), ("growth", c_int32),
                ("encoder_channels", c_int32), ("encoder_kernel_size", c_int32),
                ("encoder_stride", c_int32), ("residual_layers", c_int32),
                ("residual_dilation_factor", c_int32), ("num_head", c_int32), ("ffw_dim", c_int32),
                ("num_transformer_layers", c_int32)]

    @classmethod
    def from_config(cls, cfg):
        s = cls()
        s.n_mics, s.kernel_size, s.depth = cfg.n_mics, cfg.kernel_size, cfg.depth
        for i, v in enumerate(cfg.stride_list):
            s.stride_list[i] = v
        s.channels, s.growth = cfg.channels, int(cfg.growth)
        s.encoder_channels, s.encoder_kernel_size = cfg.encoder_channels, cfg.encoder_kernel_size
        s.encoder_stride, s.residual_layers = cfg.encoder_stride, cfg.residual_layers
        s.residual_dilation_factor, s.num_head = cfg.residual_dilation_factor, cfg.num_head
        s.ffw_dim, s.num_transformer_layers = cfg.ffw_dim, cfg.num_transformer_layers
        return s


class SepConfigC(Structure):
    _fields_ = [("n_mics", c_int32), ("max_speakers", c_int32), ("kernel_size", c_int32), ("depth", c_int32),
                ("stride_list", c_int32 * 8), ("channels", c_int32), ("growth", c_int32),
                ("encoder_channels", c_int32), ("encoder_kernel_size", c_int32), ("encoder_stride", c_int32),
                ("residual_layers", c_int32), ("residual_dilation_factor", c_int32), ("num_head", c_int32),
                ("ffw_dim", c_int32), ("bottleneck_layers", c_int32), ("bottleneck_ksize", c_int32)]

    @classmethod
    def from_config(cls, cfg):
        s = cls()
        s.n_mics, s.max_speakers, s.kernel_size, s.depth = cfg.n_mics, cfg.max_speakers, cfg.kernel_size, cfg.depth
        for i, v in enumerate(cfg.stride_list):
            s.stride_list[i] = v
        s.channels, s.growth = cfg.channels, int(cfg.growth)
        s.encoder_channels, s.encoder_kernel_size = cfg.encoder_channels, cfg.encoder_kernel_size
        s.encoder_stride, s.residual_layers = cfg.encoder_stride, cfg.residual_layers
        s.residual_dilation_factor, s.num_head = cfg.residual_dilation_factor, cfg.num_head
        s.ffw_dim, s.bottleneck_layers, s.bottleneck_ksize = cfg.ffw_dim, cfg.bottleneck_layers, cfg.bottleneck_ksize
        return s


class ConvGemmArgs(Structure):
    _fields_ = [("A", c_void_p), ("A2", c_void_p), ("Wt", c_void_p), ("bias", c_void_p),
                ("resid", c_void_p), ("mul", c_void_p), ("ln_gamma", c_void_p), ("ln_beta", c_void_p),
                ("out", c_void_p), ("stats", c_void_p),
                ("B", c_int32), ("M_out", c_int32), ("N", c_int32), ("Cin", c_int32), ("taps", c_int32),
                ("stride", c_int32), ("dil", c_int32), ("pad", c_int32), ("a_row_stride", c_int32),
                ("a_batch_stride", c_int64), ("a_len", c_int64), ("chan_mod", c_int32), ("relu", c_int32),
                ("ln_eps", c_float), ("precision", c_int32), ("w_shift", c_int32), ("Wt_hi", c_void_p),
                ("Wt_lo", c_void_p), ("Wf_hi", c_void_p), ("Wf_lo", c_void_p), ("stats_stride", c_int32),
                ("glu_raw", c_void_p), ("glu_mr", c_void_p), ("glu_gamma", c_void_p), ("glu_beta", c_void_p),
                ("glu_out", c_void_p)]


class MaskPathArgs(Structure):
    _fields_ = [("enc", ConvGemmArgs), ("ref", c_void_p), ("ref_batch_stride", c_int64), ("ref_len", c_int64),
                ("ref_hop", c_int32), ("byp_k", c_int32), ("byp_taps", c_int32), ("byp_shift", c_int32),
                ("byp_hi", c_void_p), ("byp_lo", c_void_p), ("byp_bias", c_void_p), ("dec_hi", c_void_p),
                ("dec_lo", c_void_p), ("dec_shift", c_int32), ("dec_taps", c_int32), ("taps", c_void_p)]


class ResLayerDesc(Structure):
    _fields_ = [("Wf_hi", c_void_p), ("Wf_lo", c_void_p), ("bias", c_void_p), ("ln_gamma", c_void_p),
                ("ln_beta", c_void_p), ("dil", c_int32), ("w_shift", c_int32)]


class ResStackArgs(Structure):
    _fields_ = [("x", c_void_p), ("out", c_void_p), ("B", c_int32), ("T", c_int32), ("C", c_int32), ("taps", c_int32),
                ("n_layers", c_int32), ("precision", c_int32), ("ln_eps", c_float), ("layer", ResLayerDesc * 3),
                ("glu_raw", c_void_p), ("glu_mr", c_void_p), ("glu_gamma", c_void_p), ("glu_beta", c_void_p),
                ("glu_out", c_void_p)]


SIGNATURES = {
    "asw_last_error": (c_char_p, []),
    "asw_abi_version": (c_int, []),
    "asw_profile_enable": (c_int, [c_int]),
    "asw_profile_report": (c_int, [c_char_p, c_size_t]),
    "asw_spot_create": (c_int, [POINTER(SpotConfigC), POINTER(c_void_p)]),
    "asw_spot_destroy": (None, [c_void_p]),
    "asw_spot_set_param": (c_int, [c_void_p, c_char_p, c_void_p, c_size_t]),
    "asw_spot_finalize": (c_int, [c_void_p]),
    "asw_spot_set_batch": (c_int, [c_void_p, c_int]),
    "asw_spot_set_precision": (c_int, [c_void_p, c_int]),
    "asw_spot_set_lanes": (c_int, [c_void_p, c_int]),
    "asw_split_weights_f16": (c_int, [c_void_p, c_size_t, c_void_p, c_void_p, POINTER(c_int32)]),
    "asw_pack_fragments_f16": (c_int, [c_void_p, c_int, c_int, c_void_p, c_void_p, POINTER(c_int32)]),
    "asw_spot_shift_and_sep": (c_int, [c_void_p, c_void_p, c_int, c_int, c_void_p, c_int, c_int, c_int,
                                       c_void_p, c_void_p, c_int, c_void_p]),
    "asw_spot_shift_and_sep_multi": (c_int, [c_void_p, c_void_p, c_int, c_int, c_int, c_void_p, c_void_p, c_int, c_int, c_int,
                                             c_void_p, c_void_p, c_int, c_void_p]),
    "asw_spot_forward": (c_int, [c_void_p, c_void_p, c_int, c_int, c_int, POINTER(c_float), c_void_p, c_void_p]),
    "asw_spot_set_fused_mask": (c_int, [c_void_p, c_int]),
    "asw_spot_get_tap": (c_int, [c_void_p, c_char_p, c_void_p, c_size_t, POINTER(c_size_t), c_void_p]),
    "asw_sep_create": (c_int, [POINTER(SepConfigC), POINTER(c_void_p)]),
    "asw_sep_destroy": (None, [c_void_p]),
    "asw_sep_set_param": (c_int, [c_void_p, c_char_p, c_void_p, c_size_t]),
    "asw_sep_finalize": (c_int, [c_void_p]),
    "asw_sep_set_precision": (c_int, [c_void_p, c_int]),
    "asw_sep_infer": (c_int, [c_void_p, c_void_p, c_int, c_int, c_void_p, c_int, c_void_p, c_void_p]),
    "asw_sep_forward": (c_int, [c_void_p, c_void_p, c_int, c_int, c_int, c_int, c_void_p, c_void_p]),
    "asw_sep_forward_counts": (c_int, [c_void_p, c_void_p, c_int, c_int, c_int, c_int, c_void_p, c_void_p, c_void_p]),
    "asw_sep_get_config": (c_int, [c_void_p, POINTER(SepConfigC)]),
    "asw_sep_get_tap": (c_int, [c_void_p, c_char_p, c_void_p, c_size_t, POINTER(c_size_t), c_void_p]),
    "asw_joint_shift_stats": (c_int, [c_void_p, c_int, c_int, c_void_p, c_int, c_void_p, c_void_p, c_void_p, c_void_p]),
    "asw_joint_shift_stats_scratch_doubles": (c_int, []),
    "asw_add_layernorm2": (c_int, [c_void_p, c_void_p, c_float, c_void_p, c_void_p, c_int, c_int, c_float, c_int,
                                   c_void_p, c_void_p, c_void_p]),
    "asw_glu_rows": (c_int, [c_void_p, c_long, c_int, c_void_p, c_void_p]),
    "asw_dwconv_ln_swish": (c_int, [c_void_p, c_void_p, c_void_p, c_void_p, c_void_p, c_int, c_int, c_int, c_int,
                                    c_float, c_void_p, c_void_p]),
    "asw_relpos_attention": (c_int, [c_void_p, c_void_p, c_void_p, c_void_p, c_int, c_int, c_int, c_int, c_float,
                                     c_void_p, c_void_p]),
    "asw_inter_attention": (c_int, [c_void_p, c_int, c_int, c_int, c_int, c_int, c_void_p, c_void_p]),
    "asw_shift_stats": (c_int, [c_void_p, c_int, c_int, c_void_p, c_int, c_int, c_void_p, c_void_p, c_void_p]),
    "asw_shift_norm_preproc": (c_int, [c_void_p, c_int, c_int, c_int, c_void_p, c_int, c_int, c_void_p, c_void_p,
                                       c_void_p, c_void_p, c_int, c_void_p, c_void_p, c_long, c_void_p]),
    "asw_shift_stats_multi": (c_int, [c_void_p, c_int, c_int, c_void_p, c_void_p, c_int, c_int, c_void_p, c_void_p, c_void_p]),
    "asw_shift_norm_preproc_multi": (c_int, [c_void_p, c_int, c_int, c_int, c_void_p, c_void_p, c_int, c_int, c_void_p,
                                             c_void_p, c_void_p, c_void_p, c_int, c_void_p, c_void_p, c_long, c_void_p]),
    "asw_pad_preproc": (c_int, [c_void_p, c_int, c_int, c_int, c_int, c_void_p, c_void_p, c_int, c_void_p,
                                c_void_p, c_long, c_void_p]),
    "asw_convgemm_f32": (c_int, [POINTER(ConvGemmArgs), c_void_p]),
    "asw_mask_path_f16x3": (c_int, [POINTER(MaskPathArgs), c_void_p]),
    "asw_resstack64_f16x3": (c_int, [POINTER(ResStackArgs), c_void_p]),
    "asw_convgemm_stats_tiles": (c_int, [c_int, c_int]),
    "asw_f16x3_overflow_count": (c_int, [c_int, POINTER(c_int32)]),
    "asw_gn_glu": (c_int, [c_void_p, c_void_p, c_int, c_void_p, c_void_p, c_int, c_int, c_int, c_float, c_void_p,
                           c_void_p]),
    "asw_gn_finalize": (c_int, [c_void_p, c_int, c_int, c_int, c_int, c_float, c_void_p, c_void_p]),
    "asw_attention": (c_int, [c_void_p, c_int, c_int, c_int, c_int, c_void_p, c_void_p]),
    "asw_attention_prec": (c_int, [c_void_p, c_int, c_int, c_int, c_int, c_int, c_void_p, c_void_p]),
    "asw_overlap_add_unnorm": (c_int, [c_void_p, c_int, c_int, c_int, c_int, c_int, c_int, c_int, c_int, c_float,
                                       c_void_p, c_void_p, c_void_p, c_void_p]),
    "asw_overlap_add_parts": (c_int, [c_void_p, c_int, c_int, c_int, c_int, c_int, c_int, c_int, c_int, c_int, c_float,
                                      c_void_p, c_void_p, c_void_p, c_void_p]),
    "asw_energies": (c_int, [c_void_p, c_int, c_int, c_int, c_void_p, c_void_p, c_void_p]),
    "asw_pair_sisdr": (c_int, [c_void_p, c_int, c_int, c_void_p, c_void_p]),
    "asw_center_rows": (c_int, [c_void_p, c_int, c_int, c_void_p]),
    "asw_segment_sisdr": (c_int, [c_void_p, c_int, c_int, c_void_p, c_void_p, c_int, c_void_p, c_void_p]),
    "asw_add_layernorm": (c_int, [c_void_p, c_void_p, c_void_p, c_void_p, c_int, c_int, c_float, c_void_p, c_void_p]),
    "asw_search_area": (c_int, [c_void_p, c_int, c_void_p, c_int, c_void_p, c_void_p, c_void_p, c_double, c_double,
                                POINTER(c_int), POINTER(c_void_p), POINTER(c_void_p), POINTER(c_void_p),
                                POINTER(c_void_p)]),
    "asw_free": (None, [c_void_p]),
    "asw_cube_select": (c_int, [c_void_p, c_int, c_int, c_int, c_int, c_int, c_int, c_int, c_int, c_void_p, c_void_p,
                                c_void_p, c_int64, POINTER(c_int64)]),
    "asw_cube_select_planes": (c_int, [c_void_p, c_int, c_int, c_int, c_int, c_int, c_int, c_int, c_int, c_void_p, c_void_p,
                                c_void_p, c_int64, POINTER(c_int64)]),
    "asw_srp_frames": (c_int, [c_int, c_int, c_int]),
    "asw_srp_cross_spectra": (c_int, [c_void_p, c_int, c_int, c_int, c_int, c_int, c_int, c_int, c_int, c_int,
                                      c_float, c_void_p, c_void_p, c_void_p, c_int, c_void_p, c_void_p, c_void_p]),
    "asw_srp_map": (c_int, [c_void_p, c_int, c_int, c_int, c_void_p, c_int, c_int, c_void_p, c_void_p, c_void_p,
                            c_void_p, c_void_p, c_void_p]),
    "asw_pruner_covariance": (c_int, [c_void_p, c_int, c_int, c_int, c_int, c_int, c_int, c_int, c_int, c_int,
                                      c_void_p, c_void_p, c_void_p]),
    "asw_hermitian_eigh": (c_int, [c_void_p, c_int, c_int, c_void_p, c_void_p, c_void_p]),
    "asw_music_map": (c_int, [c_void_p, c_int, c_int, c_int, c_void_p, c_int, c_void_p, c_void_p, c_void_p, c_void_p,
                              c_void_p]),
    "asw_tops_map": (c_int, [c_void_p, c_void_p, c_int, c_int, c_int, c_int, c_void_p, c_int, c_double, c_void_p,
                             c_void_p, c_void_p, c_void_p]),
    "asw_geom_lookup_planes": (c_int, [c_void_p, c_int, c_void_p, c_int, c_void_p, c_int, c_void_p, c_int, c_double, c_double,
                                       c_void_p, c_void_p]),
    "asw_geom_voxel_map": (c_int, [c_void_p, c_int, c_void_p, c_int, c_void_p, c_int, c_void_p, c_int, c_void_p, c_void_p,
                                   c_double, c_double, c_double, c_void_p, c_void_p, c_void_p, c_void_p]),
    "asw_geom_label": (c_int, [c_void_p, c_void_p, c_int, c_int, c_int, c_int, c_void_p, c_void_p, c_void_p, POINTER(c_int),
                               c_void_p]),
    "asw_geom_workspace_bytes": (c_int64, [c_int]),
    "asw_geom_compact": (c_int, [c_void_p, c_void_p, c_void_p, c_int, c_void_p, c_int, c_void_p, c_int, c_void_p, c_int,
                                 c_void_p, c_double, c_void_p, c_int64, c_void_p, c_void_p, c_void_p, c_void_p, c_void_p,
                                 c_void_p, c_void_p, c_void_p, c_void_p, POINTER(c_int), c_void_p]),
    "asw_geom_lattice_workspace_bytes": (c_int64, [c_int, c_int]),
    "asw_geom_lattice": (c_int, [c_void_p, c_int, c_int, c_int, c_int, c_void_p, c_void_p, c_void_p, c_void_p, c_double,
                                 c_void_p, c_int64, c_void_p, c_void_p, c_void_p, c_void_p, POINTER(c_int), c_void_p]),
    "asw_lattice_nms_workspace_bytes": (c_int64, [c_int, c_int]),
    "asw_lattice_nms": (c_int, [c_void_p, c_int, c_int, c_void_p, c_int, c_void_p, c_int64, c_void_p, c_void_p, c_void_p]),
}

_lib = None


def lib():
    global _lib
    if _lib is None:
        if not os.path.exists(LIB_PATH):
            raise RuntimeError(
                f"{LIB_PATH} is missing: run `python -c 'import __graft_entry__ as g; g.build()'` "
                "(hipcc --offload-arch=gfx950).  There is no CPU fallback for the hot path.")
        import torch
        L = ctypes.CDLL(LIB_PATH)
        for name, (res, args) in SIGNATURES.items():
            fn = getattr(L, name)
            fn.restype = res
            fn.argtypes = args
        _lib = L
    return _lib


_ops = None


def torch_ops():
    global _ops
    if _ops is None:
        lib()
        if not os.path.exists(OPS_PATH):
            raise RuntimeError(f"{OPS_PATH} is missing: run `python -c 'import __graft_entry__ as g; g.build()'`.  "
                               "The hot path is exposed only through these custom ops; there is no fallback.")
        import torch
        torch.ops.load_library(OPS_PATH)
        _ops = torch.ops.asw
    return _ops


def check(status: int):
    if status != 0:
        msg = lib().asw_last_error()
        raise RuntimeError(f"libasw_hip: status {status}: {msg.decode() if msg else ''}")


def ptr(t):
    return None if t is None else c_void_p(t.data_ptr())


def current_stream():
    import torch
    return c_void_p(torch.cuda.current_stream().cuda_stream)


def to_device(a, device):
    import torch
    src = torch.from_numpy(a)
    host = torch.empty(src.shape, dtype=src.dtype, pin_memory=True)
    host.copy_(src)
    return host.to(device, non_blocking=True)


def to_host(t):
    import torch
    if not t.is_cuda:
        return t.numpy()
    host = torch.empty(t.shape, dtype=t.dtype, pin_memory=True)
    host.copy_(t)
    return host.numpy()
```

### acousticswarms-speech_amd/ops.py

```python
from ctypes import byref

import torch

from .native import ConvGemmArgs, MaskPathArgs, ResStackArgs, check, current_stream, lib, ptr


def _f32(t):
    assert t.is_cuda and t.dtype == torch.float32 and t.is_contiguous(), "need contiguous float32 CUDA tensor"
    return t


def pack_conv_weight(w: torch.Tensor) -> torch.Tensor:
    N, Cin, K = w.shape
    return w.permute(0, 2, 1).reshape(N, K * Cin).contiguous()


def convgemm(A, Wt, M_out, N, Cin, taps=1, stride=1, dil=1, pad=0, bias=None, relu=False, resid=None, mul=None,
             ln=None, stats_chan_mod=0, A2=None, B=None, a_row_stride=None, a_batch_stride=None, a_len=None,
             out=None, ln_eps=1e-5, precision="f32", use_fragments=True, glu=None, glu_out=None):
    _f32(A); _f32(Wt)
    if B is None:
        B = A.shape[0]
    a_row_stride = Cin if a_row_stride is None else a_row_stride
    if a_batch_stride is None:
        a_batch_stride = A[0].numel()
    if a_len is None:
        a_len = a_batch_stride
    if out is None:
        out = torch.empty((B, M_out, N), dtype=torch.float32, device=A.device)
    stats = None
    if stats_chan_mod:
        tiles = lib().asw_convgemm_stats_tiles(M_out, N)
        stats = torch.zeros((B, tiles, 4), dtype=torch.float32, device=A.device)
    a = ConvGemmArgs()
    a.A, a.A2, a.Wt = A.data_ptr(), (A2.data_ptr() if A2 is not None else None), Wt.data_ptr()
    a.bias = bias.data_ptr() if bias is not None else None
    a.resid = resid.data_ptr() if resid is not None else None
    a.mul = mul.data_ptr() if mul is not None else None
    a.ln_gamma = ln[0].data_ptr() if ln is not None else None
    a.ln_beta = ln[1].data_ptr() if ln is not None else None
    a.out = out.data_ptr()
    a.stats = stats.data_ptr() if stats is not None else None
    a.B, a.M_out, a.N, a.Cin, a.taps, a.stride, a.dil, a.pad = B, M_out, N, Cin, taps, stride, dil, pad
    a.a_row_stride, a.a_batch_stride, a.a_len = a_row_stride, a_batch_stride, a_len
    a.chan_mod, a.relu, a.ln_eps = stats_chan_mod, int(relu), ln_eps
    if glu is not None:
        a.glu_raw, a.glu_mr, a.glu_gamma, a.glu_beta = (_f32(t).data_ptr() for t in glu)
        if glu_out is not None:
            a.glu_out = _f32(glu_out).data_ptr()
    keep = None
    if precision in ("f16x3", "f16"):
        hi, lo, shift = split_weights_f16(Wt)
        keep = (hi, lo)
        a.precision, a.w_shift, a.Wt_hi, a.Wt_lo = (1 if precision == "f16x3" else 2), shift, hi.data_ptr(), lo.data_ptr()
        if use_fragments and N % 32 == 0 and (taps * Cin) % 16 == 0:
            fh, fl, sh2 = pack_fragments_f16(Wt, N, taps * Cin)
            assert sh2 == shift
            keep = keep + (fh, fl)
            a.Wf_hi, a.Wf_lo = fh.data_ptr(), fl.data_ptr()
    check(lib().asw_convgemm_f32(byref(a), current_stream()))
    torch.cuda.current_stream().synchronize() if keep is not None else None
    return out, stats


def resstack(x, layers, taps=7, precision="f16x3", eps=1e-5, glu=None, out=None, glu_out=None):
    src = x if glu is None else glu[0]
    B, T = src.shape[0], src.shape[1]
    if out is None:
        out = torch.empty((B, T, 64), dtype=torch.float32, device=src.device)
    a = ResStackArgs()
    a.x = _f32(x).data_ptr() if x is not None else None
    a.out = out.data_ptr()
    a.B, a.T, a.C, a.taps, a.n_layers = B, T, 64, taps, len(layers)
    a.precision, a.ln_eps = (1 if precision == "f16x3" else 2), eps
    keep = []
    for i, (Wt, bias, gamma, beta, dil) in enumerate(layers):
        fh, fl, sh = pack_fragments_f16(_f32(Wt), 64, taps * 64)
        keep.append((fh, fl))
        d = a.layer[i]
        d.Wf_hi, d.Wf_lo, d.w_shift, d.dil = fh.data_ptr(), fl.data_ptr(), sh, dil
        d.bias, d.ln_gamma, d.ln_beta = _f32(bias).data_ptr(), _f32(gamma).data_ptr(), _f32(beta).data_ptr()
    if glu is not None:
        a.glu_raw, a.glu_mr, a.glu_gamma, a.glu_beta = (_f32(t).data_ptr() for t in glu)
        if glu_out is not None:
            a.glu_out = _f32(glu_out).data_ptr()
    check(lib().asw_resstack64_f16x3(byref(a), current_stream()))
    torch.cuda.current_stream().synchronize()
    return out


def pack_fragments_f16(Wt, N, K):
    import ctypes
    import numpy as np
    w = np.ascontiguousarray(Wt.detach().cpu().numpy(), dtype=np.float32).reshape(N, K)
    hi = np.empty(w.size, dtype=np.uint16)
    lo = np.empty(w.size, dtype=np.uint16)
    sh = ctypes.c_int32()
    check(lib().asw_pack_fragments_f16(ctypes.c_void_p(w.ctypes.data), N, K, ctypes.c_void_p(hi.ctypes.data),
                                       ctypes.c_void_p(lo.ctypes.data), byref(sh)))
    dev = Wt.device
    return (torch.from_numpy(hi.view(np.int16)).to(dev), torch.from_numpy(lo.view(np.int16)).to(dev), sh.value)


def split_weights_f16(Wt):
    import ctypes
    import numpy as np
    w = np.ascontiguousarray(Wt.detach().cpu().numpy(), dtype=np.float32)
    hi = np.empty(w.size, dtype=np.uint16)
    lo = np.empty(w.size, dtype=np.uint16)
    sh = ctypes.c_int32()
    check(lib().asw_split_weights_f16(ctypes.c_void_p(w.ctypes.data), w.size, ctypes.c_void_p(hi.ctypes.data),
                                      ctypes.c_void_p(lo.ctypes.data), byref(sh)))
    dev = Wt.device
    return (torch.from_numpy(hi.view(np.int16)).to(dev), torch.from_numpy(lo.view(np.int16)).to(dev), sh.value)


def gn_glu(raw, stats, gamma, beta, eps=1e-5):
    B, T, C2 = raw.shape
    C = C2 // 2
    out = torch.empty((B, T, C), dtype=torch.float32, device=raw.device)
    check(lib().asw_gn_glu(ptr(_f32(raw)), ptr(_f32(stats)), stats.shape[1], ptr(_f32(gamma)), ptr(_f32(beta)),
                           B, T, C, eps, ptr(out), current_stream()))
    return out


def gn_finalize(stats, T, C, eps=1e-5):
    B = stats.shape[0]
    mr = torch.empty((B, 4), dtype=torch.float32, device=stats.device)
    check(lib().asw_gn_finalize(ptr(_f32(stats)), stats.shape[1], B, T, C, eps, ptr(mr), current_stream()))
    return mr


def add_layernorm(x, resid, gamma, beta, eps=1e-5):
    rows, N = x.shape
    out = torch.empty_like(x)
    check(lib().asw_add_layernorm(ptr(_f32(x)), ptr(_f32(resid)), ptr(_f32(gamma)), ptr(_f32(beta)), rows, N, eps,
                                  ptr(out), current_stream()))
    return out


def attention(qkv, nhead, precision="f32"):
    B, L, d3 = qkv.shape
    d = d3 // 3
    ctx = torch.empty((B, L, d), dtype=torch.float32, device=qkv.device)
    check(lib().asw_attention_prec(ptr(_f32(qkv)), B, L, d, nhead, {"f32": 0, "f16x3": 1, "f16": 2}[precision], ptr(ctx),
                                   current_stream()))
    return ctx


def shift_stats(mix, offsets, circular=True):
    M, T = mix.shape
    N = offsets.shape[0]
    mean = torch.empty((N,), dtype=torch.float32, device=mix.device)
    std = torch.empty((N,), dtype=torch.float32, device=mix.device)
    check(lib().asw_shift_stats(ptr(_f32(mix)), M, T, ptr(offsets), N, int(circular), ptr(mean), ptr(std),
                                current_stream()))
    return mean, std


def shift_norm_preproc(mix, offsets, mean, std, w, b, T_pad, circular=True):
    M, T = mix.shape
    N = offsets.shape[0]
    C = w.shape[0]
    x0 = torch.empty((N, T_pad, C), dtype=torch.float32, device=mix.device)
    refn = torch.zeros((N, T_pad), dtype=torch.float32, device=mix.device)
    check(lib().asw_shift_norm_preproc(ptr(_f32(mix)), M, T, T_pad, ptr(offsets), N, int(circular), ptr(mean),
                                       ptr(std), ptr(_f32(w)), ptr(_f32(b)), C, ptr(x0), ptr(refn), T_pad,
                                       current_stream()))
    return x0, refn


def overlap_add_unnorm(D, taps, hop, t, trim_left, trim_right, bias, mean=None, std=None):
    B, F, ldd = D.shape
    out = torch.empty((B, t), dtype=torch.float32, device=D.device)
    check(lib().asw_overlap_add_unnorm(ptr(_f32(D)), B, F, ldd, taps, hop, t, trim_left, trim_right, float(bias),
                                       ptr(mean), ptr(std), ptr(out), current_stream()))
    return out


def overlap_add_parts(Dp, taps, hop, t, trim_left, trim_right, bias, mean=None, std=None):
    nparts, B, F, ldd = Dp.shape
    out = torch.empty((B, t), dtype=torch.float32, device=Dp.device)
    check(lib().asw_overlap_add_parts(ptr(_f32(Dp)), nparts, B, F, ldd, taps, hop, t, trim_left, trim_right,
                                      float(bias), ptr(mean), ptr(std), ptr(out), current_stream()))
    return out


def mask_path(x, ref, ref_hop, enc_w, enc_b, byp_w, byp_b, dec_w, frames, stride, pad):
    B, Tp, C = x.shape
    E, _, EK = enc_w.shape
    dev = x.device
    Wt = pack_conv_weight(enc_w).to(dev)
    fh, fl, sh = pack_fragments_f16(Wt, E, EK * C)
    wb = torch.zeros((E, 48), dtype=torch.float32)
    wb[:, :byp_w.shape[-1]] = byp_w[:, 0].cpu()
    bh, bl, bsh = pack_fragments_f16(wb.to(dev), E, 48)
    wd = torch.zeros((64, E), dtype=torch.float32)
    wd[:dec_w.shape[-1]] = dec_w[:, 0].t().cpu()
    dh, dl, dsh = pack_fragments_f16(wd.to(dev), 64, E)
    parts = torch.zeros((E // 256, B, frames, 64), dtype=torch.float32, device=dev)
    m = MaskPathArgs()
    a = m.enc
    a.A, a.bias = _f32(x).data_ptr(), (_f32(enc_b).data_ptr() if enc_b is not None else None)
    a.B, a.M_out, a.N, a.Cin, a.taps, a.stride, a.dil, a.pad = B, frames, E, C, EK, stride, 1, pad
    a.a_row_stride, a.a_batch_stride, a.a_len = C, Tp * C, Tp * C
    a.precision, a.w_shift, a.Wf_hi, a.Wf_lo = 1, sh, fh.data_ptr(), fl.data_ptr()
    m.ref, m.ref_batch_stride, m.ref_len, m.ref_hop = _f32(ref).data_ptr(), ref.shape[1], ref.shape[1], ref_hop
    m.byp_k, m.byp_taps, m.byp_shift = 48, byp_w.shape[-1], bsh
    m.byp_hi, m.byp_lo = bh.data_ptr(), bl.data_ptr()
    m.byp_bias = _f32(byp_b).data_ptr() if byp_b is not None else None
    m.dec_hi, m.dec_lo, m.dec_shift, m.dec_taps = dh.data_ptr(), dl.data_ptr(), dsh, dec_w.shape[-1]
    m.taps = parts.data_ptr()
    check(lib().asw_mask_path_f16x3(byref(m), current_stream()))
    torch.cuda.current_stream().synchronize()
    return parts


def energies(y, window=12000):
    B, T = y.shape
    scratch = torch.empty((B, T + 1), dtype=torch.float64, device=y.device)
    out = torch.empty((B, 2), dtype=torch.float64, device=y.device)
    check(lib().asw_energies(ptr(_f32(y)), B, T, window, ptr(scratch), ptr(out), current_stream()))
    return out


def pair_sisdr(y):
    n, T = y.shape
    out = torch.empty((n, n), dtype=torch.float64, device=y.device)
    check(lib().asw_pair_sisdr(ptr(_f32(y)), n, T, ptr(out), current_stream()))
    return out


def srp_cross_spectra(mix, twiddle, pair_i, pair_j, nbins, window, step, n_windows, nfft, hop, tol=1e-8):
    M, T = mix.shape
    P = pair_i.shape[0]
    nb_pad = twiddle.shape[0] // 2
    assert twiddle.shape == (2 * nb_pad, nfft), "twiddle must be [2*nb_pad, nfft]"
    for t in (pair_i, pair_j):
        assert t.is_cuda and t.dtype == torch.int32 and t.is_contiguous() and t.numel() == P, "pair tables: int32 [P]"
    F = lib().asw_srp_frames(window, nfft, hop)
    xf = torch.empty((M, max(F, 1), 2 * nb_pad), dtype=torch.float32, device=mix.device)
    cc = torch.full((n_windows, nbins, P, 2), float("nan"), dtype=torch.float32, device=mix.device)
    check(lib().asw_srp_cross_spectra(ptr(_f32(mix)), M, T, window, step, n_windows, nfft, hop, nbins, nb_pad, tol,
                                      ptr(_f32(twiddle)), ptr(pair_i), ptr(pair_j), P, ptr(xf), ptr(cc),
                                      current_stream()))
    return cc


def srp_map(cc, tau, omega, pair_i, pair_j):
    n_windows, nbins, P, _ = cc.shape
    G, M = tau.shape
    for t, dt, n in ((tau, torch.float64, G * M), (omega, torch.float64, nbins), (pair_i, torch.int32, P),
                     (pair_j, torch.int32, P)):
        assert t.is_cuda and t.dtype == dt and t.is_contiguous() and t.numel() == n, "srp_map: operand dtype / size"
    part = torch.empty((8 * 8 * G,), dtype=torch.float32, device=cc.device)
    out = torch.empty((G,), dtype=torch.float32, device=cc.device)
    check(lib().asw_srp_map(ptr(_f32(cc)), n_windows, nbins, P, ptr(tau), G, M, ptr(omega), ptr(pair_i), ptr(pair_j),
                            ptr(part), ptr(out), current_stream()))
    return out


def joint_shift_stats(mix, offsets):
    M, T = mix.shape
    S = offsets.shape[0]
    scratch = torch.empty((lib().asw_joint_shift_stats_scratch_doubles(),), dtype=torch.float64, device=mix.device)
    mean = torch.empty((S,), dtype=torch.float32, device=mix.device)
    std = torch.empty((S,), dtype=torch.float32, device=mix.device)
    check(lib().asw_joint_shift_stats(ptr(_f32(mix)), M, T, ptr(offsets), S, ptr(scratch), ptr(mean), ptr(std),
                                      current_stream()))
    return mean, std


def add_layernorm2(x, y=None, alpha=1.0, gamma=None, beta=None, eps=1e-5, act=0, want_sum=False, want_ln=True):
    rows, N = x.shape
    s = torch.empty_like(x) if want_sum else None
    o = torch.empty_like(x) if want_ln else None
    check(lib().asw_add_layernorm2(ptr(_f32(x)), ptr(y), float(alpha), ptr(gamma), ptr(beta), rows, N, eps, act, ptr(s),
                                   ptr(o), current_stream()))
    return s, o


def glu_rows(raw):
    rows, C2 = raw.shape
    out = torch.empty((rows, C2 // 2), dtype=torch.float32, device=raw.device)
    check(lib().asw_glu_rows(ptr(_f32(raw)), rows, C2 // 2, ptr(out), current_stream()))
    return out


def dwconv_ln_swish(u, w, bias, gamma, beta, eps=1e-5):
    BS, L, d = u.shape
    K = w.shape[-1]
    wT = w.reshape(d, K).t().contiguous()
    out = torch.empty_like(u)
    check(lib().asw_dwconv_ln_swish(ptr(_f32(u)), ptr(_f32(wT)), ptr(_f32(bias)), ptr(_f32(gamma)), ptr(_f32(beta)),
                                    BS, L, d, K, eps, ptr(out), current_stream()))
    return out


def relpos_attention(qkv, P, bias_u, bias_v, nhead, scale):
    BS, L, d3 = qkv.shape
    d = d3 // 3
    ctx = torch.empty((BS, L, d), dtype=torch.float32, device=qkv.device)
    check(lib().asw_relpos_attention(ptr(_f32(qkv)), ptr(_f32(P)), ptr(_f32(bias_u)), ptr(_f32(bias_v)), BS, L, d, nhead,
                                     float(scale), ptr(ctx), current_stream()))
    return ctx


def inter_attention(qkv, nhead):
    NB, S, L, d3 = qkv.shape
    d = d3 // 3
    ctx = torch.empty((NB, S, L, d), dtype=torch.float32, device=qkv.device)
    check(lib().asw_inter_attention(ptr(_f32(qkv)), NB, S, L, d, nhead, ptr(ctx), current_stream()))
    return ctx


def f16x3_overflow_count(reset=True) -> int:
    import ctypes
    c = ctypes.c_int32()
    check(lib().asw_f16x3_overflow_count(int(reset), byref(c)))
    return int(c.value) & 0xFFFFFFFF
```

### acousticswarms-speech_amd/spot.py

```python
from collections import OrderedDict
from ctypes import byref, c_size_t, c_void_p

import numpy as np

from . import native
from .config import FULL, SpotConfig, spot_param_shapes


def offsets_from_patches(patch_list, n_pairs: int) -> np.ndarray:
    if len(patch_list) == 0:
        return np.zeros((0, n_pairs), dtype=np.int32)
    offs = np.stack([np.asarray(getattr(p, "sample_offset", p), dtype=np.float64) for p in patch_list])
    if offs.shape[1] != n_pairs:
        raise RuntimeError(f"candidate has {offs.shape[1]} offsets, mixture has {n_pairs + 1} channels")
    return np.rint(offs.astype(np.float32)).astype(np.int32)


class SpotModel:
    PRECISIONS = {"f32": 0, "f16x3": 1, "f16": 2}

    def __init__(self, cfg: SpotConfig = FULL, state_dict=None, batch_size: int = 32, precision: str = "f32",
                 lanes: int = 1):
        if precision not in self.PRECISIONS:
            raise RuntimeError(f"precision must be one of {list(self.PRECISIONS)}")
        self.cfg = cfg
        self.precision = precision
        self.batch_size = batch_size
        self.lanes = int(lanes)
        self.device = None
        self._h = None
        self._sd = None
        self.last_waveforms = None
        if state_dict is not None:
            self.load_state_dict(state_dict)

    def load_state_dict(self, sd, strict: bool = True):
        import contextlib
        want = OrderedDict(spot_param_shapes(self.cfg))
        clean = OrderedDict()
        for k, v in sd.items():
            a = v.detach().cpu().numpy() if hasattr(v, "detach") else np.asarray(v)
            clean[k] = np.ascontiguousarray(a, dtype=np.float32)
        missing = [k for k in want if k not in clean]
        extra = [k for k in clean if k not in want]
        if strict and (missing or extra):
            raise RuntimeError(f"Error(s) in loading state_dict: missing {missing[:3]} unexpected {extra[:3]}")
        for k, shp in want.items():
            if k in clean and tuple(clean[k].shape) != tuple(shp):
                raise RuntimeError(f"size mismatch for {k}: {tuple(clean[k].shape)} vs {tuple(shp)}")
        self._sd = clean
        if self._h is not None:
            import torch
            with (torch.cuda.device(self.device) if self.device is not None else contextlib.nullcontext()):
                self._upload()
        return self

    def _upload(self):
        L = native.lib()
        for k, a in self._sd.items():
            native.check(L.asw_spot_set_param(self._h, k.encode(), c_void_p(a.ctypes.data), a.size))
        native.check(L.asw_spot_finalize(self._h))

    def to(self, device=None):
        import torch
        if device is None:
            return self
        device = torch.device(device)
        if device.type != "cuda":
            raise RuntimeError("SpotModel runs only on an MI355X (device 'cuda'); there is no CPU path")
        if not torch.cuda.is_available():
            raise RuntimeError("no HIP device visible: the spot hot path has no CPU fallback")
        if device.index is None:
            device = torch.device("cuda", torch.cuda.current_device())
        L = native.lib()
        with torch.cuda.device(device):
            if self._h is not None:
                L.asw_spot_destroy(self._h)
                self._h = None
            h = c_void_p()
            cc = native.SpotConfigC.from_config(self.cfg)
            native.check(L.asw_spot_create(byref(cc), byref(h)))
            self._h = h
            native.check(L.asw_spot_set_batch(self._h, int(self.batch_size)))
            native.check(L.asw_spot_set_precision(self._h, self.PRECISIONS[self.precision]))
            native.check(L.asw_spot_set_lanes(self._h, self.lanes))
            self.device = device
            if self._sd is not None:
                self._upload()
        return self

    def eval(self):
        return self

    def set_precision(self, precision: str):
        if precision not in self.PRECISIONS:
            raise RuntimeError(f"precision must be one of {list(self.PRECISIONS)}")
        self.precision = precision
        if self._h is not None:
            native.check(native.lib().asw_spot_set_precision(self._h, self.PRECISIONS[precision]))

    def set_lanes(self, lanes: int):
        self.lanes = int(lanes)
        if self._h is not None:
            native.check(native.lib().asw_spot_set_lanes(self._h, self.lanes))

    def set_batch_size(self, b: int):
        self.batch_size = int(b)
        if self._h is not None:
            native.check(native.lib().asw_spot_set_batch(self._h, int(b)))

    def __del__(self):
        try:
            if self._h is not None:
                native.lib().asw_spot_destroy(self._h)
        except Exception:
            pass

    def _need(self):
        if self._h is None:
            raise RuntimeError("SpotModel.to('cuda') must be called before inference")
        if self._sd is None:
            raise RuntimeError("SpotModel has no weights: call load_state_dict()")

    def shift_and_sep_device(self, mix_dev, offsets_dev, strict: int = 0, want_wave: bool = True,
                             want_energy: bool = False, window: int = 12000, circular: bool = True):
        import torch
        self._need()
        M, T = mix_dev.shape
        N = offsets_dev.shape[0]
        assert mix_dev.dtype == torch.float32 and mix_dev.is_contiguous() and mix_dev.is_cuda
        assert offsets_dev.dtype == torch.int32 and offsets_dev.is_contiguous() and offsets_dev.is_cuda
        wave, en = native.torch_ops().spot_shift_and_sep(self._h.value, mix_dev, offsets_dev, int(strict), bool(circular),
                                                         bool(want_wave), bool(want_energy), int(window))
        return (wave if want_wave else None), (en if want_energy else None)

    def shift_and_sep_device_multi(self, mix_stack, offsets_dev, mix_index_dev, strict: int = 0, want_wave: bool = True,
                                   want_energy: bool = False, window: int = 12000, circular: bool = True):
        import torch
        self._need()
        assert mix_stack.dim() == 3 and mix_stack.dtype == torch.float32 and mix_stack.is_contiguous() and mix_stack.is_cuda
        assert offsets_dev.dtype == torch.int32 and offsets_dev.is_contiguous() and offsets_dev.is_cuda
        assert mix_index_dev.dtype == torch.int32 and mix_index_dev.is_contiguous() and mix_index_dev.is_cuda
        wave, en = native.torch_ops().spot_shift_and_sep_multi(self._h.value, mix_stack, offsets_dev, mix_index_dev,
                                                               int(strict), bool(circular), bool(want_wave),
                                                               bool(want_energy), int(window))
        return (wave if want_wave else None), (en if want_energy else None)

    def shift_and_sep(self, input_channels, patch_list, Strict: int = 0, save_input: bool = False) -> np.ndarray:
        import torch
        self._need()
        if save_input:
            raise RuntimeError("save_input=True is a debugging path of the reference that materialises every "
                               "shifted mixture; it is not provided (the shifted tensor never exists here)")
        mix = torch.as_tensor(input_channels)
        T = mix.shape[-1]
        if len(patch_list) == 0:
            return np.empty((0, T), dtype=np.float32)
        offs = offsets_from_patches(patch_list, mix.shape[0] - 1)
        mix_d = mix.to(self.device, dtype=torch.float32).contiguous()
        off_d = torch.from_numpy(offs).to(self.device)
        wave, _ = self.shift_and_sep_device(mix_d, off_d, Strict, want_wave=True)
        return native.to_host(wave)

    def shift_and_score(self, input_channels, patch_list, Strict: int = 0, window: int = 12000,
                        keep_waveforms: bool = True) -> np.ndarray:
        import torch
        self._need()
        mix = torch.as_tensor(input_channels)
        if len(patch_list) == 0:
            self.last_waveforms = None
            return np.empty((0, 2), dtype=np.float64)
        offs = offsets_from_patches(patch_list, mix.shape[0] - 1)
        mix_d = mix.to(self.device, dtype=torch.float32).contiguous()
        off_d = torch.from_numpy(offs).to(self.device)
        wave, en = self.shift_and_sep_device(mix_d, off_d, Strict, want_wave=keep_waveforms, want_energy=True,
                                             window=window)
        self.last_waveforms = wave
        return en.cpu().numpy()

    def shift_and_sep_resident(self, input_channels, patch_list, Strict: int = 0, window: int = 12000,
                               device_energies: bool = False):
        import torch
        self._need()
        mix = torch.as_tensor(input_channels)
        offs = offsets_from_patches(patch_list, mix.shape[0] - 1)
        mix_d = mix.to(self.device, dtype=torch.float32).contiguous()
        if device_energies:
            off_d = torch.from_numpy(offs).pin_memory().to(self.device, non_blocking=True)
        else:
            off_d = torch.from_numpy(offs).to(self.device)
        wave, en = self.shift_and_sep_device(mix_d, off_d, Strict, want_wave=True, want_energy=True, window=window)
        native.torch_ops().center_rows_(wave)
        return wave, (en if device_energies else en.cpu().numpy())

    def pair_sisdr(self, waves):
        return native.torch_ops().pair_sisdr(waves.contiguous()).cpu().numpy()

    def segment_sisdr(self, waves, segments):
        import torch
        n, T = waves.shape
        cnt = np.array([len(s) for s in segments], dtype=np.int32)
        kmax = max(1, int(cnt.max()) if n else 1)
        seg = np.zeros((n, kmax, 2), dtype=np.int32)
        for i, sl in enumerate(segments):
            for k, (a, b) in enumerate(sl):
                if not (0 <= a <= b <= T):
                    raise RuntimeError(f"segment [{a},{b}) of waveform {i} lies outside [0,{T}]")
                seg[i, k] = (a, b)
        out = native.torch_ops().segment_sisdr(waves.contiguous(), torch.from_numpy(seg).to(waves.device),
                                               torch.from_numpy(cnt).to(waves.device))
        return out.cpu().numpy(), cnt

    def forward(self, mix, window_embedding):
        import torch
        self._need()
        mix = torch.as_tensor(mix).to(self.device, dtype=torch.float32).contiguous()
        wemb = torch.as_tensor(window_embedding, dtype=torch.float32).cpu().numpy().reshape(mix.shape[0], 2)
        B, M, t = mix.shape
        out = torch.empty((B, 1, t), dtype=torch.float32, device=self.device)
        keys = {}
        for i, row in enumerate(map(tuple, wemb)):
            keys.setdefault(row, []).append(i)
        ops = native.torch_ops()
        for row, idx in keys.items():
            whole = len(idx) == B
            y = ops.spot_forward(self._h.value, mix if whole else mix[idx].contiguous(), float(row[0]), float(row[1]))
            if whole:
                return y.view(B, 1, t)
            out.view(B, t)[idx] = y
        return out

    __call__ = forward

    def set_fused_mask(self, on: bool = True):
        self._need()
        native.check(native.lib().asw_spot_set_fused_mask(self._h, int(bool(on))))
        return self

    def get_tap(self, name: str, shape=None):
        import torch
        n = c_size_t()
        L = native.lib()
        native.check(L.asw_spot_get_tap(self._h, name.encode(), None, 0, byref(n), None))
        buf = torch.empty((n.value,), dtype=torch.float32, device=self.device)
        with torch.cuda.device(self.device):
            native.check(L.asw_spot_get_tap(self._h, name.encode(), native.ptr(buf), n.value, byref(n),
                                            native.current_stream()))
        return buf if shape is None else buf.view(*shape)
```

### include/asw_hip.h

```cpp
#ifndef ASW_HIP_H
#define ASW_HIP_H

#include <stddef.h>
#include <stdint.h>

#ifdef __cplusplus
extern "C" {
#endif

typedef enum asw_status {
  ASW_OK = 0,
  ASW_ERR_ARG = -1,
  ASW_ERR_HIP = -2,
  ASW_ERR_NOMEM = -3,
  ASW_ERR_STATE = -4
} asw_status;

const char* asw_last_error(void);
int asw_abi_version(void);

int asw_profile_enable(int on);
int asw_profile_report(char* buf, size_t cap);

typedef struct asw_spot_config {
  int32_t n_mics;
  int32_t kernel_size;
  int32_t depth;
  int32_t stride_list[8];
  int32_t channels;
  int32_t growth;
  int32_t encoder_channels;
  int32_t encoder_kernel_size;
  int32_t encoder_stride;
  int32_t residual_layers;
  int32_t residual_dilation_factor;
  int32_t num_head;
  int32_t ffw_dim;
  int32_t num_transformer_layers;
} asw_spot_config;

typedef struct asw_spot asw_spot;

int asw_spot_create(const asw_spot_config* cfg, asw_spot** out);
void asw_spot_destroy(asw_spot* m);

int asw_spot_set_param(asw_spot* m, const char* key, const float* host_data, size_t numel);
int asw_spot_finalize(asw_spot* m);

int asw_spot_set_batch(asw_spot* m, int batch);

int asw_spot_set_lanes(asw_spot* m, int lanes);

int asw_spot_set_precision(asw_spot* m, int precision);

int asw_spot_shift_and_sep(asw_spot* m, const float* mix, int M, int T,
                           const int32_t* offsets, int N, int strict, int circular,
                           float* out_wave, double* out_energy, int energy_window,
                           void* stream);

int asw_spot_shift_and_sep_multi(asw_spot* m, const float* mix, int K, int M, int T, const int32_t* offsets,
                                 const int32_t* mix_index, int N, int strict, int circular, float* out_wave,
                                 double* out_energy, int energy_window, void* stream);

int asw_spot_forward(asw_spot* m, const float* mix_norm, int B, int M, int t,
                     const float* window_embedding_host, float* out, void* stream);

int asw_spot_set_fused_mask(asw_spot* m, int on);

int asw_spot_get_tap(asw_spot* m, const char* name, float* dst, size_t capacity, size_t* numel,
                     void* stream);

typedef struct asw_sep_config {
  int32_t n_mics;
  int32_t max_speakers;
  int32_t kernel_size;
  int32_t depth;
  int32_t stride_list[8];
  int32_t channels;
  int32_t growth;
  int32_t encoder_channels;
  int32_t encoder_kernel_size;
  int32_t encoder_stride;
  int32_t residual_layers;
  int32_t residual_dilation_factor;
  int32_t num_head;
  int32_t ffw_dim;
  int32_t bottleneck_layers;
  int32_t bottleneck_ksize;
} asw_sep_config;

typedef struct asw_sep asw_sep;

int asw_sep_create(const asw_sep_config* cfg, asw_sep** out);
void asw_sep_destroy(asw_sep* m);
int asw_sep_set_param(asw_sep* m, const char* key, const float* host_data, size_t numel);
int asw_sep_finalize(asw_sep* m);
int asw_sep_set_precision(asw_sep* m, int precision);

int asw_sep_infer(asw_sep* m, const float* mix, int M, int T, const int32_t* offsets, int S, float* out,
                  void* stream);

int asw_sep_forward(asw_sep* m, const float* mix_norm, int B, int S, int M, int t, float* out, void* stream);
int asw_sep_forward_counts(asw_sep* m, const float* mix_norm, int B, int S, int M, int t, const int32_t* counts,
                           float* out, void* stream);
int asw_sep_get_config(const asw_sep* m, asw_sep_config* out);

int asw_sep_get_tap(asw_sep* m, const char* name, float* dst, size_t capacity, size_t* numel, void* stream);

int asw_joint_shift_stats(const float* mix, int M, int T, const int32_t* offsets, int S, double* scratch,
                          float* mean, float* std, void* stream);
int asw_joint_shift_stats_scratch_doubles(void);

int asw_add_layernorm2(const float* x, const float* y, float alpha, const float* gamma, const float* beta,
                       int rows, int N, float eps, int act, float* sum_out, float* ln_out, void* stream);

int asw_glu_rows(const float* raw, long rows, int C, float* out, void* stream);

int asw_dwconv_ln_swish(const float* u, const float* wT, const float* bias, const float* gamma, const float* beta,
                        int BS, int L, int d, int K, float eps, float* out, void* stream);

int asw_relpos_attention(const float* qkv, const float* P, const float* bias_u, const float* bias_v, int BS, int L,
                         int d, int nhead, float scale, float* ctx, void* stream);

int asw_inter_attention(const float* qkv, int NB, int S, int L, int d, int nhead, float* ctx, void* stream);


int asw_shift_stats(const float* mix, int M, int T, const int32_t* offsets, int N,
                    int circular, float* mean, float* std, void* stream);

int asw_shift_norm_preproc(const float* mix, int M, int T, int T_pad, const int32_t* offsets,
                           int N, int circular, const float* mean, const float* std,
                           const float* w, const float* b, int C, float* x0, float* refn,
                           long refn_stride, void* stream);

int asw_shift_stats_multi(const float* mix, int M, int T, const int32_t* offsets, const int32_t* mix_index, int N,
                          int circular, float* mean, float* std, void* stream);
int asw_shift_norm_preproc_multi(const float* mix, int M, int T, int T_pad, const int32_t* offsets,
                                 const int32_t* mix_index, int N, int circular, const float* mean, const float* std,
                                 const float* w, const float* b, int C, float* x0, float* refn, long refn_stride,
                                 void* stream);

int asw_pad_preproc(const float* x, int B, int M, int t, int T_pad, const float* w,
                    const float* b, int C, float* x0, float* refn, long refn_stride,
                    void* stream);

typedef struct asw_convgemm_args {
  const float* A;
  const float* A2;
  const float* Wt;
  const float* bias;
  const float* resid;
  const float* mul;
  const float* ln_gamma;
  const float* ln_beta;
  float* out;
  float* stats;
  int32_t B, M_out, N, Cin, taps, stride, dil, pad;
  int32_t a_row_stride;
  int64_t a_batch_stride;
  int64_t a_len;
  int32_t chan_mod;
  int32_t relu;
  float ln_eps;
  int32_t precision;
  int32_t w_shift;
  const void* Wt_hi;
  const void* Wt_lo;
  const void* Wf_hi;
  const void* Wf_lo;
  int32_t stats_stride;
  const float* glu_raw;
  const float* glu_mr;
  const float* glu_gamma;
  const float* glu_beta;
  float* glu_out;
} asw_convgemm_args;
int asw_pack_fragments_f16(const float* Wt, int N, int K, uint16_t* hi, uint16_t* lo, int32_t* w_shift);
int asw_convgemm_f32(const asw_convgemm_args* args, void* stream);
typedef struct asw_maskpath_args {
  asw_convgemm_args enc;
  const float* ref;
  int64_t ref_batch_stride;
  int64_t ref_len;
  int32_t ref_hop;
  int32_t byp_k;
  int32_t byp_taps;
  int32_t byp_shift;
  const void* byp_hi;
  const void* byp_lo;
  const float* byp_bias;
  const void* dec_hi;
  const void* dec_lo;
  int32_t dec_shift;
  int32_t dec_taps;
  float* taps;
} asw_maskpath_args;
int asw_mask_path_f16x3(const asw_maskpath_args* args, void* stream);
typedef struct asw_reslayer_desc {
  const void* Wf_hi;
  const void* Wf_lo;
  const float* bias;
  const float* ln_gamma;
  const float* ln_beta;
  int32_t dil;
  int32_t w_shift;
} asw_reslayer_desc;
typedef struct asw_resstack_args {
  const float* x;
  float* out;
  int32_t B, T, C, taps, n_layers;
  int32_t precision;
  float ln_eps;
  asw_reslayer_desc layer[3];
  const float* glu_raw;
  const float* glu_mr;
  const float* glu_gamma;
  const float* glu_beta;
  float* glu_out;
} asw_resstack_args;
int asw_resstack64_f16x3(const asw_resstack_args* args, void* stream);
int asw_split_weights_f16(const float* w, size_t n, uint16_t* hi, uint16_t* lo, int32_t* w_shift);
int asw_f16x3_overflow_count(int reset, uint32_t* count);
int asw_convgemm_stats_tiles(int M_out, int N);

int asw_gn_glu(const float* raw, const float* stats, int n_partials, const float* gamma,
               const float* beta, int B, int T, int C, float eps, float* out, void* stream);
int asw_gn_finalize(const float* stats, int n_partials, int B, int T, int C, float eps, float* mr, void* stream);

int asw_attention(const float* qkv, int B, int L, int d, int nhead, float* ctx, void* stream);
int asw_attention_prec(const float* qkv, int B, int L, int d, int nhead, int precision, float* ctx, void* stream);

int asw_overlap_add_unnorm(const float* D, int B, int F, int ldd, int taps, int hop,
                           int t, int trim_left, int trim_right, float bias, const float* mean,
                           const float* std, float* out, void* stream);
int asw_overlap_add_parts(const float* D, int nparts, int B, int F, int ldd, int taps, int hop,
                          int t, int trim_left, int trim_right, float bias, const float* mean,
                          const float* std, float* out, void* stream);

int asw_energies(const float* y, int B, int T, int window, double* scratch, double* out,
                 void* stream);

int asw_add_layernorm(const float* x, const float* resid, const float* gamma, const float* beta,
                      int rows, int N, float eps, float* out, void* stream);

int asw_center_rows(float* y, int B, int T, void* stream);

int asw_pair_sisdr(const float* y, int n, int T, double* out, void* stream);

int asw_segment_sisdr(const float* y, int n, int T, const int32_t* segments, const int32_t* seg_count,
                      int kmax, double* out, void* stream);

int asw_search_area(const double* points, int n_pts, const double* mic, int M, double* offset,
                    double* width, const double* ub, double sound_speed, double fs, int* n_children,
                    double** child_offset, double** child_width, int** child_count, int** child_index);
void asw_free(void* p);

int asw_cube_select(const double* offsets, int ny, int nx, int nz, int P, int y0, int y1, int x0, int x1,
                    const double* lo, const double* hi, int32_t* out_idx, int64_t cap, int64_t* count);
int asw_cube_select_planes(const double* planes, int ny, int nx, int nz, int P, int y0, int y1, int x0, int x1,
                    const double* lo, const double* hi, int32_t* out_idx, int64_t cap, int64_t* count);

int asw_srp_frames(int window, int nfft, int hop);
int asw_srp_cross_spectra(const float* mix, int M, int T, int window, int step, int n_windows,
                          int nfft, int hop, int nbins, int nb_pad, float tol,
                          const float* twiddle, const int32_t* pair_i, const int32_t* pair_j,
                          int P, float* xf_scratch, float* cc, void* stream);
int asw_srp_map(const float* cc, int n_windows, int nbins, int P, const double* tau, int G, int M,
                const double* omega, const int32_t* pair_i, const int32_t* pair_j,
                float* part_scratch, float* out, void* stream);

int asw_pruner_covariance(const float* mix, int M, int T, int window, int step, int n_windows,
                          int nfft, int hop, int bin0, int nbins, double* cov, double* magsum,
                          void* stream);
int asw_hermitian_eigh(const double* a, int n, int M, double* evals, double* evecs, void* stream);
int asw_music_map(const double* evecs, int n_windows, int nbins, int M, const double* tau, int G,
                  const double* omega, double* p_scratch, double* max_scratch, float* out,
                  void* stream);
int asw_tops_map(const double* evecs, const double* magsum, int n_windows, int nbins, int bin0,
                 int M, const double* delta, int G, double coef, double* q_scratch,
                 int32_t* max_bin, float* out, void* stream);

int asw_geom_lookup_planes(const double* ys, int ny, const double* xs, int nx, const double* zs, int nz,
                           const double* mics, int M, double C, double FS, double* planes, void* stream);
int asw_geom_voxel_map(const double* xs, int Lx, const double* ys, int Ly, const double* zs, int Lz,
                       const double* mics, int M, const double* border, const double* centre, double C,
                       double FS, double resolution, int32_t* q, uint8_t* valid, double* dis_matrix,
                       void* stream);
int asw_geom_label(const int32_t* q, const uint8_t* valid, int Lx, int Ly, int Lz, int P,
                   uint32_t* adj_scratch, int32_t* flag_scratch, int32_t* labels, int* sweeps, void* stream);
int64_t asw_geom_workspace_bytes(int n_voxels);
int asw_geom_compact(const int32_t* labels, const int32_t* q, const double* xs, int Lx, const double* ys, int Ly,
                     const double* zs, int Lz, const double* mics, int M, const double* centre, double C,
                     void* workspace, int64_t workspace_bytes, int32_t* power_index, int32_t* valid_flat,
                     int32_t* valid_cid, int32_t* members, int32_t* bounds, int32_t* offsets, double* centres,
                     double* tau, double* delta, int* counts, void* stream);
int64_t asw_geom_lattice_workspace_bytes(int n_points, int P);
int asw_geom_lattice(const double* planes, int P, int ny, int nx, int nz, const double* xs, const double* ys,
                     const double* zs, const double* border, double width, void* workspace,
                     int64_t workspace_bytes, int32_t* cells, int32_t* bounds, int32_t* members, double* centres,
                     int* counts, void* stream);
int64_t asw_lattice_nms_workspace_bytes(int N, int P);
int asw_lattice_nms(const int32_t* cells, int N, int P, const double* scores, int radius, void* workspace,
                    int64_t workspace_bytes, int32_t* best, int32_t* degree, void* stream);

#ifdef __cplusplus
}
#endif
#endif
```

Baseline: 2352 candidates/s.

## Fold preproc 1x1 conv into first encoder residual layer via composed weights

The 7-mic to 64-channel preprocessing conv is composed algebraically with the first encoder residual conv. A new prep kernel writes compact 8-lane f16 hi/lo source planes: the normalised shifted mics plus a constant-1 bias lane. A source-fed variant of the fused res-stack kernel then computes layer 0 straight from those planes, and rebuilds the residual term through a second small MFMA with the preproc weights. This removes the write and re-read of the 64-channel preproc activation tensor for each candidate. In exchange it adds weight composition at load time, pre_up/pre_down scaling, and a restricted set of shapes where the path applies.

```diff
diff --git a/acousticswarms-speech_amd/csrc/model_common.h b/acousticswarms-speech_amd/csrc/model_common.h
--- a/acousticswarms-speech_amd/csrc/model_common.h
+++ b/acousticswarms-speech_amd/csrc/model_common.h
@@ -150,24 +150,33 @@
   return true;
 }
 
+inline size_t resstack_fuse_count(const std::vector<ResLayer>& res, size_t j, int K) {
+  static const bool nofuse = getenv("ASW_RESSTACK_NOFUSE") != nullptr;
+  size_t n = 1;
+  int halo = 0;
+  while (!nofuse && j + n < res.size() && n < 3) {
+    const int pad = res[j + n].dil * (K - 1) / 2;
+    if (halo + pad > 64) break;
+    halo += pad;
+    ++n;
+  }
+  return n;
+}
+
+struct SrcFeed { const void* hi; const void* lo; const WBuf* comp; const WBuf* pre; };
+
 inline int run_res(const std::vector<ResLayer>& res, int prec, int B, int T, int ch, int K, float* x, float* p, float* q,
-            float** final_out, hipStream_t s, const GluSrc* glu = nullptr) {
+            float** final_out, hipStream_t s, const GluSrc* glu = nullptr, const SrcFeed* feed = nullptr) {
   const float* in = glu ? glu->raw : x;
   float* outb = p;
+  if (feed && !(resstack_ok(res, prec, ch, K) && prec == 1 && resstack_fuse_count(res, 0, K) == 2))
+    return asw::set_error(ASW_ERR_STATE, "run_res: the source-fed form needs the fused f16x3 pair");
   if (resstack_ok(res, prec, ch, K)) {
-    static const bool nofuse = getenv("ASW_RESSTACK_NOFUSE") != nullptr;
     size_t j = 0;
     while (j < res.size()) {
-      size_t n = 1;
-      int halo = 0;
-      while (!nofuse && j + n < res.size() && n < 3) {
-        const int pad = res[j + n].dil * (K - 1) / 2;
-        if (halo + pad > 64) break;
-        halo += pad;
-        ++n;
-      }
+      const size_t n = resstack_fuse_count(res, j, K);
       asw_resstack_args a = {};
-      a.x = (glu && j == 0) ? nullptr : in;
+      a.x = ((glu || feed) && j == 0) ? nullptr : in;
       a.out = outb;
       a.B = B; a.T = T; a.C = ch; a.taps = K; a.n_layers = (int)n; a.precision = prec; a.ln_eps = 1e-5f;
       for (size_t i = 0; i < n; ++i) {
@@ -177,6 +186,11 @@
       }
       if (glu && j == 0) {
         a.glu_raw = glu->raw; a.glu_mr = glu->mr; a.glu_gamma = glu->gamma; a.glu_beta = glu->beta; a.glu_out = glu->side_out;
+      }
+      if (feed && j == 0) {
+        a.src_hi = feed->hi; a.src_lo = feed->lo;
+        a.layer[0].Wf_hi = feed->comp->fhi; a.layer[0].Wf_lo = feed->comp->flo; a.layer[0].w_shift = feed->comp->shift;
+        a.pre_hi = feed->pre->fhi; a.pre_lo = feed->pre->flo; a.pre_shift = feed->pre->shift;
       }
       int rc = asw_resstack64_f16x3(&a, s);
       if (rc) return rc;
@@ -276,6 +290,7 @@
   int B, T, Tp, F, RL;
   std::vector<int> Tl;
   float *mean, *stdv, *refn;
+  uint16_t *src_hi = nullptr, *src_lo = nullptr;
   std::vector<float*> X, Pb, Qb, raw_dn, raw_up, st_dn, st_up, mr_dn, mr_up;
   float *Y, *D, *ywave;
 };
@@ -288,12 +303,15 @@
   int device = 0;
   int precision = 0;
   bool fuse_mask = true;
+  bool want_src = false;
+  bool src_stack = true;
 
   std::vector<int> enc_cin, enc_cout;
   std::vector<int> dec_cin, dec_cout, dec_stride;
   int stride_product = 1;
 
   DevBuf pre_w, pre_b;
+  WBuf src_wt, src_pre;
   std::vector<EncBlock> enc;
   std::vector<DecBlock> dec;
   WBuf byp_wt, mask_wt, dec_wt;
@@ -396,6 +414,14 @@
       UP(enc[i].gn_g, P(p + ".norm1.weight"));
       UP(enc[i].gn_b, P(p + ".norm1.bias"));
     }
+    if (want_src && tc.channels == 64 && tc.n_mics <= 7 && K <= 7 && enc[0].res[0].wt.fhi) {
+      std::vector<float> pre16((size_t)64 * 16), comp((size_t)64 * 64);
+      if ((rc = asw_compose_source_weights(P("encoder.module_list.0.res.seq.0.conv.weight").data(), P("preproc.weight").data(),
+                                           P("preproc.bias").data(), tc.n_mics, K, comp.data(), pre16.data())))
+        return rc;
+      if ((rc = src_wt.upload_gemm(comp, 64, 64))) return rc;
+      if ((rc = src_pre.upload_gemm(pre16, 64, 16))) return rc;
+    }
     for (int i = 0; i < tc.depth; ++i) {
       const std::string p = "decoder.module_list." + std::to_string(i);
       if ((rc = pack_res_layers(raw, p, dec_cout[i], K, RL, RD, dec[i].res))) return rc;
@@ -462,6 +488,11 @@
     return fuse_mask && precision >= 1 && tc.encoder_channels % 256 == 0 && tc.channels % 32 == 0 &&
            tc.encoder_kernel_size <= 48 && tc.encoder_stride % 4 == 0 && byp_wt48.fhi && dec_wt.fhi && mask_wt.fhi;
   }
+  bool src_path() const {
+    return want_src && src_stack && precision == 1 && src_wt.fhi && src_pre.fhi && !enc.empty() &&
+           resstack_ok(enc[0].res, precision, enc_cin[0], tc.kernel_size) &&
+           resstack_fuse_count(enc[0].res, 0, tc.kernel_size) == 2;
+  }
   void layout_levels(int B, int T, Arena& a, TrunkPlan& pl) const {
     const int depth = tc.depth, EK = tc.encoder_kernel_size, ES = tc.encoder_stride;
     pl.B = B; pl.T = T;
@@ -473,6 +504,10 @@
     pl.mean = a.take<float>(B);
     pl.stdv = a.take<float>(B);
     pl.refn = a.take<float>((size_t)B * pl.RL);
+    if (want_src) {
+      pl.src_hi = a.take<uint16_t>((size_t)B * pl.Tp * 8);
+      pl.src_lo = a.take<uint16_t>((size_t)B * pl.Tp * 8);
+    }
     pl.X.resize(depth + 1); pl.Pb.resize(depth); pl.Qb.resize(depth);
     pl.raw_dn.resize(depth); pl.raw_up.resize(depth); pl.st_dn.resize(depth); pl.st_up.resize(depth);
     pl.mr_up.resize(depth); pl.mr_dn.resize(depth);
@@ -504,17 +539,18 @@
     pl.ywave = a.take<float>((size_t)pl.B * pl.T);
   }
 
-  int encode(TrunkPlan& pl, const GatedConvs& g, hipStream_t s) {
+  int encode(TrunkPlan& pl, const GatedConvs& g, hipStream_t s, bool src0 = false) {
     const int B = pl.B, K = tc.kernel_size;
     taps.clear();
-    taps["preproc"] = {pl.X[0], (size_t)B * pl.Tl[0] * tc.channels};
+    if (!src0) taps["preproc"] = {pl.X[0], (size_t)B * pl.Tl[0] * tc.channels};
     int rc;
     GluSrc src = {};
+    const SrcFeed feed = {pl.src_hi, pl.src_lo, &src_wt, &src_pre};
     bool glu = false;
     for (int i = 0; i < tc.depth; ++i) {
       float* r = nullptr;
       if ((rc = run_res(enc[i].res, precision, B, pl.Tl[i], enc_cin[i], K, pl.X[i], pl.Pb[i], pl.Qb[i], &r, s,
-                        glu ? &src : nullptr)))
+                        glu ? &src : nullptr, (src0 && i == 0) ? &feed : nullptr)))
         return rc;
       asw_convgemm_args a = {};
       a.A = r; g.down_wt[i].bind(a, precision); a.bias = enc[i].bias.p; a.out = pl.raw_dn[i]; a.stats = pl.st_dn[i];
diff --git a/acousticswarms-speech_amd/csrc/prep_kernels.hip b/acousticswarms-speech_amd/csrc/prep_kernels.hip
--- a/acousticswarms-speech_amd/csrc/prep_kernels.hip
+++ b/acousticswarms-speech_amd/csrc/prep_kernels.hip
@@ -1,4 +1,5 @@
 #include "asw_common.h"
+#include "mfma_util.h"
 
 namespace {
 
@@ -129,6 +130,58 @@
   }
 }
 
+__global__ __launch_bounds__(256) void src_planes_kernel(const float* __restrict__ srcs, int M, int T, int T_pad,
+                                                         const int32_t* __restrict__ offsets,
+                                                         const int32_t* __restrict__ mix_index, int circular,
+                                                         const float* __restrict__ mean, const float* __restrict__ stdv,
+                                                         asw_mfma::half8* __restrict__ src_hi,
+                                                         asw_mfma::half8* __restrict__ src_lo, float* __restrict__ refn,
+                                                         long refn_stride) {
+  constexpr int ROWS = 256;
+  __shared__ int off[8];
+  __shared__ float vs[ROWS * 7];
+  const int n = blockIdx.y;
+  const float* __restrict__ src = srcs + (mix_index ? (long)mix_index[n] * M * T : 0);
+  if (threadIdx.x < M) {
+    int o = 0;
+    if (threadIdx.x > 0) {
+      o = offsets[(long)n * (M - 1) + threadIdx.x - 1];
+      if (circular) { o %= T; if (o < 0) o += T; }
+    }
+    off[threadIdx.x] = o;
+  }
+  __syncthreads();
+  const int pad = T_pad - T;
+  const float mu = mean[n], sg = stdv[n];
+  const int row0 = blockIdx.x * ROWS;
+  for (int it = threadIdx.x; it < ROWS * M; it += blockDim.x) {
+    const int m = it / ROWS, r = it - m * ROWS;
+    const int tp = row0 + r;
+    float x = 0.f;
+    if (tp >= pad && tp < T_pad) {
+      int i = tp - pad + off[m];
+      if (circular) { if (i >= T) i -= T; x = src[(long)m * T + i]; }
+      else x = (i >= 0 && i < T) ? src[(long)m * T + i] : 0.f;
+      x = (quant16(x) - mu) / sg;
+    }
+    vs[r * M + m] = x;
+  }
+  __syncthreads();
+  const int r = threadIdx.x, tp = row0 + r;
+  if (tp >= T_pad) return;
+  float u[8];
+#pragma unroll
+  for (int m = 0; m < 7; ++m) u[m] = m < M ? vs[r * M + m] : 0.f;
+  u[7] = 1.0f;
+  asw_mfma::half4 h0, l0, h1, l1;
+  asw_mfma::split4t<3>(make_float4(u[0], u[1], u[2], u[3]), h0, l0);
+  asw_mfma::split4t<3>(make_float4(u[4], u[5], u[6], u[7]), h1, l1);
+  const long o = (long)n * T_pad + tp;
+  src_hi[o] = asw_mfma::half8{h0[0], h0[1], h0[2], h0[3], h1[0], h1[1], h1[2], h1[3]};
+  src_lo[o] = asw_mfma::half8{l0[0], l0[1], l0[2], l0[3], l1[0], l1[1], l1[2], l1[3]};
+  refn[(long)n * refn_stride + tp] = u[0];
+}
+
 }
 
 extern "C" int asw_shift_stats(const float* mix, int M, int T, const int32_t* offsets, int N, int circular,
@@ -174,6 +227,22 @@
   return ASW_OK;
 }
 
+extern "C" int asw_shift_norm_src_multi(const float* mix, int M, int T, int T_pad, const int32_t* offsets,
+                                        const int32_t* mix_index, int N, int circular, const float* mean, const float* std,
+                                        void* src_hi, void* src_lo, float* refn, long refn_stride, void* stream) {
+  ASW_CHECK_ARG(refn_stride >= T_pad, "shift_norm_src: refn_stride < T_pad");
+  ASW_CHECK_ARG(mix && offsets && mean && std && src_hi && src_lo && refn, "shift_norm_src: null pointer");
+  ASW_CHECK_ARG(M >= 1 && M <= 7 && T >= 1 && T_pad >= T, "shift_norm_src: bad shape M=%d T=%d T_pad=%d (M <= 7)", M, T, T_pad);
+  if (N == 0) return ASW_OK;
+  dim3 grid(asw::cdiv(T_pad, 256), N);
+  asw::ProfScope prof(asw::as_stream(stream), "preproc_src", 0.0, (double)M * T * 4 + (double)N * T_pad * (32 + 4));
+  hipLaunchKernelGGL(src_planes_kernel, grid, dim3(256), 0, asw::as_stream(stream), mix, M, T, T_pad, offsets, mix_index,
+                     circular, mean, std, reinterpret_cast<asw_mfma::half8*>(src_hi), reinterpret_cast<asw_mfma::half8*>(src_lo),
+                     refn, refn_stride);
+  ASW_LAUNCH_CHECK();
+  return ASW_OK;
+}
+
 extern "C" int asw_pad_preproc(const float* x, int B, int M, int t, int T_pad, const float* w, const float* b,
                                int C, float* x0, float* refn, long refn_stride, void* stream) {
   ASW_CHECK_ARG(refn_stride >= T_pad, "pad_preproc: refn_stride < T_pad");
diff --git a/acousticswarms-speech_amd/csrc/resstack.hip b/acousticswarms-speech_amd/csrc/resstack.hip
--- a/acousticswarms-speech_amd/csrc/resstack.hip
+++ b/acousticswarms-speech_amd/csrc/resstack.hip
@@ -36,15 +36,28 @@
   const float* glu_gamma;
   const float* glu_beta;
   float* glu_out;
+  const half8* src_h;
+  const half8* src_l;
+  const half8* Pre_h;
+  const half8* Pre_l;
+  float pre_up, pre_down;
   int B, T, taps, ntile, BM, img_rows;
   float eps;
   LayerDev L[MAXL];
 };
 
-template <int NL, int NW, int TM, int PH, bool POLY, bool GLU, int NTERM, int QD>
+__device__ __forceinline__ __amdgpu_buffer_rsrc_t src_rsrc(const half8* base, long rows) {
+  return __builtin_amdgcn_make_buffer_rsrc(const_cast<half8*>(base), 0, (int)(rows * 16), 0x00020000);
+}
+__device__ __forceinline__ half8 src_load(__amdgpu_buffer_rsrc_t r, int row) {
+  return __builtin_bit_cast(half8, __builtin_amdgcn_raw_buffer_load_b128(r, row >= 0 ? row * 16 : (int)0x80000000, 0, 0));
+}
+
+template <int NL, int NW, int TM, int PH, bool POLY, bool GLU, int NTERM, int QD, bool SRC = false>
 __global__ __launch_bounds__(64 * NW) __attribute__((amdgpu_waves_per_eu(TM >= 4 ? 1 : 2)))
 void resstack64_kernel(const KArgs p) {
   static_assert(!POLY || NL == 1, "polyphase row sets: single layers only");
+  static_assert(!SRC || (!POLY && !GLU && NTERM == 3), "source-fed layer 0: contiguous tiles, f16x3");
   static_assert(QD == 2 || QD == 4, "weight prefetch depth in k-steps");
   constexpr int NTHR = 64 * NW, SROWS = NTHR / 16;
   constexpr int R0 = 32 * NW * TM;
@@ -68,12 +81,14 @@
   const int R_img = POLY ? PH * RJ : R0 + 2 * pad0;
 
   RS_MARK(t_start);
-  for (int i = tid; i < NL * 3 * 16; i += NTHR) {
-    const int li = i / 48, w = (i - li * 48) / 16, c4 = i & 15;
-    const float* src = w == 0 ? p.L[li].bias : w == 1 ? p.L[li].gamma : p.L[li].beta;
-    reinterpret_cast<float4*>(tab)[i] = *reinterpret_cast<const float4*>(src + c4 * 4);
-  }
-  {
+  if constexpr (!SRC) {
+    for (int i = tid; i < NL * 3 * 16; i += NTHR) {
+      const int li = i / 48, w = (i - li * 48) / 16, c4 = i & 15;
+      const float* src = w == 0 ? p.L[li].bias : w == 1 ? p.L[li].gamma : p.L[li].beta;
+      reinterpret_cast<float4*>(tab)[i] = *reinterpret_cast<const float4*>(src + c4 * 4);
+    }
+  }
+  if constexpr (!SRC) {
     const __amdgpu_buffer_rsrc_t rX = GLU ? act_rsrc(p.glu_raw + (long)b * T * 2 * C, (long)T * 2 * C)
                                           : act_rsrc(p.x + (long)b * T * C, (long)T * C);
     const int srow = tid >> 4, sc4 = tid & 15;
@@ -133,7 +148,7 @@
       }
     }
   }
-  __syncthreads();
+  if constexpr (!SRC) __syncthreads();
   RS_MARK(t_staged);
 #ifdef ASW_PHASE_TIMING
   unsigned long long t_marks[2 * MAXL + 1];
@@ -171,6 +186,69 @@
 #pragma unroll
       for (int i = 0; i < NF; ++i) { acc[i][0] = a[i][0]; acc[i][1] = a[i][1]; }
     };
+    if constexpr (SRC && li == 0) {
+      const __amdgpu_buffer_rsrc_t rH = src_rsrc(p.src_h + (long)b * T, T), rL = src_rsrc(p.src_l + (long)b * T, T);
+      const int g0 = m0 - Ld.halo - Ld.pad + wid * TM * 32 + (lane & 31);
+      half8 xh[4][TM], xl[4][TM], rh[TM], rl[TM];
+#pragma unroll
+      for (int ks = 0; ks < 4; ++ks)
+#pragma unroll
+        for (int i = 0; i < TM; ++i) {
+          xh[ks][i] = src_load(rH, g0 + i * 32 + 2 * ks + h);
+          xl[ks][i] = src_load(rL, g0 + i * 32 + 2 * ks + h);
+        }
+#pragma unroll
+      for (int i = 0; i < TM; ++i) {
+        rh[i] = src_load(rH, g0 + i * 32 + Ld.pad);
+        rl[i] = src_load(rL, g0 + i * 32 + Ld.pad);
+      }
+      half8 wh[2][2], wl[2][2];
+      auto wload = [&](auto kgc, int slot) {
+        constexpr int kg = decltype(kgc)::value;
+#pragma unroll
+        for (int cb = 0; cb < 2; ++cb) {
+          if constexpr (kg < 4) frag_load<3>(Ld.Wh, Ld.Wl, (long)kg * 2 + cb, lane, wh[slot][cb], wl[slot][cb]);
+          else frag_load<3>(p.Pre_h, p.Pre_l, (long)cb, lane, wh[slot][cb], wl[slot][cb]);
+        }
+      };
+      wload(std::integral_constant<int, 0>{}, 0);
+      wload(std::integral_constant<int, 1>{}, 1);
+      for (int i = tid; i < NL * 3 * 16; i += NTHR) {
+        const int lj = i / 48, w = (i - lj * 48) / 16, c4 = i & 15;
+        const float* src = w == 0 ? p.L[lj].bias : w == 1 ? p.L[lj].gamma : p.L[lj].beta;
+        reinterpret_cast<float4*>(tab)[i] = *reinterpret_cast<const float4*>(src + c4 * 4);
+      }
+      __syncthreads();
+      auto kstep = [&](auto ksc) {
+        constexpr int ks = decltype(ksc)::value;
+#pragma unroll
+        for (int i = 0; i < TM; ++i)
+#pragma unroll
+          for (int cb = 0; cb < 2; ++cb) mma3<3, true>(acc[i][cb], xh[ks][i], xl[ks][i], wh[ks & 1][cb], wl[ks & 1][cb]);
+        if constexpr (ks + 2 <= 4) wload(std::integral_constant<int, ks + 2>{}, ks & 1);
+        __builtin_amdgcn_sched_barrier(0);
+      };
+      kstep(std::integral_constant<int, 0>{});
+      kstep(std::integral_constant<int, 1>{});
+      kstep(std::integral_constant<int, 2>{});
+      kstep(std::integral_constant<int, 3>{});
+      const float* tb0 = tab;
+#pragma unroll
+      for (int i = 0; i < TM; ++i) {
+#pragma unroll
+        for (int cb = 0; cb < 2; ++cb)
+#pragma unroll
+          for (int q = 0; q < 4; ++q) {
+            const float4 bi = *reinterpret_cast<const float4*>(tb0 + cb * 32 + q * 8 + h * 4);
+            const float bv[4] = {bi.x, bi.y, bi.z, bi.w};
+#pragma unroll
+            for (int j = 0; j < 4; ++j)
+              acc[i][cb][q * 4 + j] = fmaxf(acc[i][cb][q * 4 + j] * Ld.scale + bv[j], 0.f) * p.pre_up;
+          }
+#pragma unroll
+        for (int cb = 0; cb < 2; ++cb) mma3<3, true>(acc[i][cb], rh[i], rl[i], wh[0][cb], wl[0][cb]);
+      }
+    } else {
     if (nf >= TM) run(std::integral_constant<int, TM>{});
     else if constexpr (TM > 1) {
       if (nf == 1) run(std::integral_constant<int, 1>{});
@@ -179,6 +257,7 @@
         if (nf == 3) run(std::integral_constant<int, 3>{});
       }
     }
+    }
 #ifdef ASW_PHASE_TIMING
     {
       float sink = acc[0][0][0];
@@ -205,8 +284,13 @@
             const float bv[4] = {bi.x, bi.y, bi.z, bi.w};
 #pragma unroll
             for (int j = 0; j < 4; ++j) {
-              float v = fmaxf(acc[i][cb][q * 4 + j] * Ld.scale + bv[j], 0.f);
-              v += (float)rh[j] + (float)rl[j];
+              float v;
+              if constexpr (SRC && li == 0) {
+                v = acc[i][cb][q * 4 + j] * p.pre_down;
+              } else {
+                v = fmaxf(acc[i][cb][q * 4 + j] * Ld.scale + bv[j], 0.f);
+                v += (float)rh[j] + (float)rl[j];
+              }
               acc[i][cb][q * 4 + j] = v;
               s += v;
             }
@@ -234,7 +318,7 @@
       }
     }
     if constexpr (!last) {
-      __syncthreads();
+      if constexpr (!(SRC && li == 0)) __syncthreads();
 #pragma unroll
       for (int i = 0; i < TM; ++i) {
         if (i < nf) {
@@ -311,15 +395,21 @@
 #endif
 }
 
-template <int NL, int NW, int TM, int PH, bool POLY, bool GLU, int QD>
+template <int NL, int NW, int TM, int PH, bool POLY, bool GLU, int QD, bool SRC = false>
 int launch_stack(const KArgs& k, int precision, size_t smem, double flops, const char* tag, hipStream_t s) {
   char nm[128], detail[48] = "";
-  snprintf(nm, sizeof nm, "resstack64<%s,%dx%d%s%s>", tag, NW, TM, POLY ? (PH == 1 ? ",poly1" : PH == 2 ? ",poly2" : ",poly4") : "",
-           GLU ? ",glu" : "");
+  snprintf(nm, sizeof nm, "resstack64<%s,%dx%d%s%s%s>", tag, NW, TM, POLY ? (PH == 1 ? ",poly1" : PH == 2 ? ",poly2" : ",poly4") : "",
+           GLU ? ",glu" : "", SRC ? ",src" : "");
   if (asw::prof_detail()) snprintf(detail, sizeof detail, "[B%d M%d d%d]", k.B, k.T, k.L[0].dil);
+  if constexpr (SRC) {
+    return asw::launch_pair<resstack64_kernel<NL, NW, TM, PH, POLY, GLU, 3, QD, true>, resstack64_kernel<NL, NW, TM, PH, POLY, GLU, 3, QD, true>>(
+        1, dim3(xcd_grid_run(k.B * k.ntile)), dim3(64 * NW), smem, 160 * 1024, nm, detail, flops,
+        (double)k.B * k.T * (32 + C * 4), s, k);
+  } else {
   return asw::launch_pair<resstack64_kernel<NL, NW, TM, PH, POLY, GLU, 1, QD>, resstack64_kernel<NL, NW, TM, PH, POLY, GLU, 3, QD>>(
       precision, dim3(xcd_grid_run(k.B * k.ntile)), dim3(64 * NW), smem, 160 * 1024, nm, detail, flops,
       (double)k.B * k.T * C * 4 * (GLU ? 3 : 2), s, k);
+  }
 }
 
 template <int NW, int TM>
@@ -355,6 +445,10 @@
   const size_t smem = (size_t)rows * RS + (size_t)a.n_layers * 3 * 64 * sizeof(float);
   ASW_CHECK_ARG(smem <= 160 * 1024, "resstack: image of %d rows exceeds LDS (dilation %d x %d taps too wide for a contiguous tile)",
                 rows, dil0, a.taps);
+  if (k.src_h) {
+    ASW_CHECK_ARG(k.L[0].nfrag == NW * TM, "resstack: source-fed layer 0 computes %d of %d fragments", k.L[0].nfrag, NW * TM);
+    return launch_stack<2, NW, TM, 1, false, false, 4, true>(k, a.precision, smem, flops, "2", s);
+  }
   switch (a.n_layers) {
     case 1: return glu ? launch_stack<1, NW, TM, 1, false, true, 4>(k, a.precision, smem, flops, "1", s)
                        : launch_stack<1, NW, TM, 1, false, false, 4>(k, a.precision, smem, flops, "1", s);
@@ -377,6 +471,26 @@
   return ASW_OK;
 }
 #endif
+
+extern "C" int asw_compose_source_weights(const float* wc, const float* wpre, const float* bpre, int M, int taps, float* comp,
+                                          float* pre16) {
+  ASW_CHECK_ARG(wc && wpre && bpre && comp && pre16, "compose_source_weights: null pointer");
+  ASW_CHECK_ARG(M >= 1 && M <= 7 && taps >= 1 && taps <= 7, "compose_source_weights: M=%d taps=%d (at most 7 each)", M, taps);
+  for (int i = 0; i < C * 16; ++i) pre16[i] = 0.f;
+  for (int i = 0; i < C * 64; ++i) comp[i] = 0.f;
+  for (int c = 0; c < C; ++c) {
+    for (int m = 0; m < M; ++m) pre16[c * 16 + m] = wpre[c * M + m];
+    pre16[c * 16 + 7] = bpre[c];
+  }
+  for (int n = 0; n < C; ++n)
+    for (int k = 0; k < taps; ++k)
+      for (int j = 0; j < 8; ++j) {
+        double acc = 0.0;
+        for (int c = 0; c < C; ++c) acc += (double)wc[((size_t)n * C + c) * taps + k] * (double)pre16[c * 16 + j];
+        comp[n * 64 + k * 8 + j] = (float)acc;
+      }
+  return ASW_OK;
+}
 
 extern "C" int asw_resstack64_f16x3(const asw_resstack_args* args, void* stream) {
   ASW_CHECK_ARG(args != nullptr, "resstack: null args");
@@ -387,7 +501,7 @@
   ASW_CHECK_ARG(a.taps >= 3 && a.taps <= 15 && a.taps % 2 == 1, "resstack: taps=%d (odd, 3..15)", a.taps);
   ASW_CHECK_ARG(a.precision == 1 || a.precision == 2, "resstack: precision 1 (f16x3) or 2 (single-pass f16)");
   ASW_CHECK_ARG(a.B > 0 && a.B <= (1 << 20) && a.T > 0 && (int64_t)a.T * 2 * C < ((int64_t)1 << 29), "resstack: bad B / T");
-  ASW_CHECK_ARG(a.out && (a.x || a.glu_raw), "resstack: null tensor");
+  ASW_CHECK_ARG(a.out && (a.x || a.glu_raw || a.src_hi), "resstack: null tensor");
   const bool glu = a.glu_raw != nullptr;
   if (glu) ASW_CHECK_ARG(a.glu_mr && a.glu_gamma && a.glu_beta, "resstack: GroupNorm + GLU on load needs the statistics / affine arrays");
   KArgs k = {};
@@ -405,6 +519,15 @@
     L.scale = ldexpf(1.0f, -d.w_shift);
     halo += L.pad;
   }
-  const double flops = 2.0 * a.B * (double)a.T * C * C * a.taps * a.n_layers;
+  double flops = 2.0 * a.B * (double)a.T * C * C * a.taps * a.n_layers;
+  if (a.src_hi) {
+    ASW_CHECK_ARG(a.src_lo && a.pre_hi && a.pre_lo && !a.x && !glu, "resstack: the source-fed form takes src_hi / src_lo / pre_hi / pre_lo and no x");
+    ASW_CHECK_ARG(a.precision == 1 && a.n_layers == 2 && a.taps <= 7 && a.layer[0].dil == 1,
+                  "resstack: source-fed layer 0 is f16x3, two layers, dilation 1, at most 7 taps");
+    k.src_h = reinterpret_cast<const half8*>(a.src_hi); k.src_l = reinterpret_cast<const half8*>(a.src_lo);
+    k.Pre_h = reinterpret_cast<const half8*>(a.pre_hi); k.Pre_l = reinterpret_cast<const half8*>(a.pre_lo);
+    k.pre_up = ldexpf(1.0f, a.pre_shift); k.pre_down = ldexpf(1.0f, -a.pre_shift);
+    flops = 2.0 * a.B * (double)a.T * C * (64 + 16 + C * a.taps);
+  }
   return dispatch<4, 2>(a, k, glu, flops, s);
 }
diff --git a/acousticswarms-speech_amd/csrc/spot_model.hip b/acousticswarms-speech_amd/csrc/spot_model.hip
--- a/acousticswarms-speech_amd/csrc/spot_model.hip
+++ b/acousticswarms-speech_amd/csrc/spot_model.hip
@@ -27,6 +27,7 @@
   hipStream_t side = nullptr;
   hipEvent_t ev_fork = nullptr, ev_join = nullptr;
 
+  asw_spot() { want_src = true; }
   ~asw_spot() {
     for (char* w : ws) if (w) (void)hipFree(w);
     if (side) (void)hipStreamDestroy(side);
@@ -141,10 +142,10 @@
 }
 
 int run_network(asw_spot* m, Plan& pl, GateSet* gs, const float* mean, const float* stdv, float* out_wave,
-                hipStream_t s) {
+                hipStream_t s, bool src0 = false) {
   const asw_spot_config& c = m->cfg;
   int rc;
-  if ((rc = m->encode(pl, *gs, s))) return rc;
+  if ((rc = m->encode(pl, *gs, s, src0))) return rc;
   const int L = pl.Tl[c.depth], d = m->enc_cout.back(), rows = pl.B * L;
   const float* h = pl.X[c.depth];
   for (int l = 0; l < c.num_transformer_layers; ++l) {
@@ -265,6 +266,7 @@
     ASW_HIP(hipStreamWaitEvent(m->side, m->ev_fork, 0));
   }
   const int C = m->cfg.channels, pad_l = m->cfg.encoder_kernel_size / 2;
+  const bool src0 = m->src_path();
   auto batches = [&]() -> int {
     int k = 0;
     for (int i0 = 0; i0 < N; i0 += Bmax, ++k) {
@@ -277,11 +279,16 @@
       ASW_HIP(hipMemsetAsync(p.refn, 0, (size_t)B * p.RL * sizeof(float), q));
       int r;
       if ((r = asw_shift_stats_multi(mix, M, T, off, mi, B, circular, p.mean, p.stdv, q))) return r;
-      if ((r = asw_shift_norm_preproc_multi(mix, M, T, p.Tp, off, mi, B, circular, p.mean, p.stdv, m->pre_w.p, m->pre_b.p, C,
-                                            p.X[0], p.refn + pad_l, p.RL, q)))
+      if (src0) {
+        if ((r = asw_shift_norm_src_multi(mix, M, T, p.Tp, off, mi, B, circular, p.mean, p.stdv, p.src_hi, p.src_lo,
+                                          p.refn + pad_l, p.RL, q)))
+          return r;
+      } else if ((r = asw_shift_norm_preproc_multi(mix, M, T, p.Tp, off, mi, B, circular, p.mean, p.stdv, m->pre_w.p,
+                                                   m->pre_b.p, C, p.X[0], p.refn + pad_l, p.RL, q))) {
         return r;
+      }
       float* y = out_wave ? out_wave + (size_t)i0 * T : p.ywave;
-      if ((r = run_network(m, p, gs, p.mean, p.stdv, y, q))) return r;
+      if ((r = run_network(m, p, gs, p.mean, p.stdv, y, q, src0))) return r;
       if (out_energy && (r = asw_energies(y, B, T, energy_window, p.escr, out_energy + (size_t)i0 * 2, q))) return r;
     }
     return ASW_OK;
@@ -335,6 +342,12 @@
   return ASW_OK;
 }
 
+extern "C" int asw_spot_set_source_stack(asw_spot* m, int on) {
+  ASW_CHECK_ARG(m, "set_source_stack: null model handle");
+  m->src_stack = on != 0;
+  return ASW_OK;
+}
+
 extern "C" int asw_spot_get_tap(asw_spot* m, const char* name, float* dst, size_t capacity, size_t* numel,
                                 void* stream) {
   return get_tap(m, "get_tap", name, dst, capacity, numel, stream);
diff --git a/acousticswarms-speech_amd/native.py b/acousticswarms-speech_amd/native.py
--- a/acousticswarms-speech_amd/native.py
+++ b/acousticswarms-speech_amd/native.py
@@ -135,7 +135,8 @@
     _fields_ = [("x", c_void_p), ("out", c_void_p), ("B", c_int32), ("T", c_int32), ("C", c_int32), ("taps", c_int32),
                 ("n_layers", c_int32), ("precision", c_int32), ("ln_eps", c_float), ("layer", ResLayerDesc * 3),
                 ("glu_raw", c_void_p), ("glu_mr", c_void_p), ("glu_gamma", c_void_p), ("glu_beta", c_void_p),
-                ("glu_out", c_void_p)]
+                ("glu_out", c_void_p), ("src_hi", c_void_p), ("src_lo", c_void_p), ("pre_hi", c_void_p), ("pre_lo", c_void_p),
+                ("pre_shift", c_int32)]
 
 
 SIGNATURES = {
@@ -158,6 +159,7 @@
                                              c_void_p, c_void_p, c_int, c_void_p]),
     "asw_spot_forward": (c_int, [c_void_p, c_void_p, c_int, c_int, c_int, POINTER(c_float), c_void_p, c_void_p]),
     "asw_spot_set_fused_mask": (c_int, [c_void_p, c_int]),
+    "asw_spot_set_source_stack": (c_int, [c_void_p, c_int]),
     "asw_spot_get_tap": (c_int, [c_void_p, c_char_p, c_void_p, c_size_t, POINTER(c_size_t), c_void_p]),
     "asw_sep_create": (c_int, [POINTER(SepConfigC), POINTER(c_void_p)]),
     "asw_sep_destroy": (None, [c_void_p]),
@@ -185,11 +187,14 @@
     "asw_shift_stats_multi": (c_int, [c_void_p, c_int, c_int, c_void_p, c_void_p, c_int, c_int, c_void_p, c_void_p, c_void_p]),
     "asw_shift_norm_preproc_multi": (c_int, [c_void_p, c_int, c_int, c_int, c_void_p, c_void_p, c_int, c_int, c_void_p,
                                              c_void_p, c_void_p, c_void_p, c_int, c_void_p, c_void_p, c_long, c_void_p]),
+    "asw_shift_norm_src_multi": (c_int, [c_void_p, c_int, c_int, c_int, c_void_p, c_void_p, c_int, c_int, c_void_p,
+                                         c_void_p, c_void_p, c_void_p, c_void_p, c_long, c_void_p]),
     "asw_pad_preproc": (c_int, [c_void_p, c_int, c_int, c_int, c_int, c_void_p, c_void_p, c_int, c_void_p,
                                 c_void_p, c_long, c_void_p]),
     "asw_convgemm_f32": (c_int, [POINTER(ConvGemmArgs), c_void_p]),
     "asw_mask_path_f16x3": (c_int, [POINTER(MaskPathArgs), c_void_p]),
     "asw_resstack64_f16x3": (c_int, [POINTER(ResStackArgs), c_void_p]),
+    "asw_compose_source_weights": (c_int, [c_void_p, c_void_p, c_void_p, c_int, c_int, c_void_p, c_void_p]),
     "asw_convgemm_stats_tiles": (c_int, [c_int, c_int]),
     "asw_f16x3_overflow_count": (c_int, [c_int, POINTER(c_int32)]),
     "asw_gn_glu": (c_int, [c_void_p, c_void_p, c_int, c_void_p, c_void_p, c_int, c_int, c_int, c_float, c_void_p,
diff --git a/acousticswarms-speech_amd/ops.py b/acousticswarms-speech_amd/ops.py
--- a/acousticswarms-speech_amd/ops.py
+++ b/acousticswarms-speech_amd/ops.py
@@ -89,6 +89,39 @@
     return out
 
 
+def resstack_src(src_hi, src_lo, pre_w, pre_b, layers, taps=7, eps=1e-5, out=None):
+    import ctypes
+    import numpy as np
+    B, T = src_hi.shape[0], src_hi.shape[1]
+    dev = src_hi.device
+    if out is None:
+        out = torch.empty((B, T, 64), dtype=torch.float32, device=dev)
+    M = pre_w.shape[1]
+    wc = np.ascontiguousarray(layers[0][0].detach().cpu().numpy(), dtype=np.float32)
+    wp = np.ascontiguousarray(pre_w.detach().cpu().numpy(), dtype=np.float32).reshape(64, M)
+    bp = np.ascontiguousarray(pre_b.detach().cpu().numpy(), dtype=np.float32)
+    comp, pre16 = np.empty((64, 64), dtype=np.float32), np.empty((64, 16), dtype=np.float32)
+    check(lib().asw_compose_source_weights(ctypes.c_void_p(wc.ctypes.data), ctypes.c_void_p(wp.ctypes.data),
+                                           ctypes.c_void_p(bp.ctypes.data), M, taps, ctypes.c_void_p(comp.ctypes.data),
+                                           ctypes.c_void_p(pre16.ctypes.data)))
+    a = ResStackArgs()
+    a.out = out.data_ptr()
+    a.B, a.T, a.C, a.taps, a.n_layers, a.precision, a.ln_eps = B, T, 64, taps, len(layers), 1, eps
+    keep = []
+    for i, (w, bias, gamma, beta, dil) in enumerate(layers):
+        Wt = torch.from_numpy(comp).to(dev) if i == 0 else pack_conv_weight(w).to(dev)
+        fh, fl, sh = pack_fragments_f16(Wt, 64, Wt.shape[1])
+        keep.append((fh, fl))
+        d = a.layer[i]
+        d.Wf_hi, d.Wf_lo, d.w_shift, d.dil = fh.data_ptr(), fl.data_ptr(), sh, dil
+        d.bias, d.ln_gamma, d.ln_beta = _f32(bias).data_ptr(), _f32(gamma).data_ptr(), _f32(beta).data_ptr()
+    ph, pl, psh = pack_fragments_f16(torch.from_numpy(pre16).to(dev), 64, 16)
+    a.src_hi, a.src_lo, a.pre_hi, a.pre_lo, a.pre_shift = src_hi.data_ptr(), src_lo.data_ptr(), ph.data_ptr(), pl.data_ptr(), psh
+    check(lib().asw_resstack64_f16x3(byref(a), current_stream()))
+    torch.cuda.current_stream().synchronize()
+    return out
+
+
 def pack_fragments_f16(Wt, N, K):
     import ctypes
     import numpy as np
@@ -168,6 +201,17 @@
                                        ptr(std), ptr(_f32(w)), ptr(_f32(b)), C, ptr(x0), ptr(refn), T_pad,
                                        current_stream()))
     return x0, refn
+
+
+def shift_norm_src(mix, offsets, mean, std, T_pad, circular=True):
+    M, T = mix.shape
+    N = offsets.shape[0]
+    hi = torch.empty((N, T_pad, 8), dtype=torch.float16, device=mix.device)
+    lo = torch.empty((N, T_pad, 8), dtype=torch.float16, device=mix.device)
+    refn = torch.zeros((N, T_pad), dtype=torch.float32, device=mix.device)
+    check(lib().asw_shift_norm_src_multi(ptr(_f32(mix)), M, T, T_pad, ptr(offsets), None, N, int(circular), ptr(mean),
+                                         ptr(std), ptr(hi), ptr(lo), ptr(refn), T_pad, current_stream()))
+    return hi, lo, refn
 
 
 def overlap_add_unnorm(D, taps, hop, t, trim_left, trim_right, bias, mean=None, std=None):
diff --git a/acousticswarms-speech_amd/spot.py b/acousticswarms-speech_amd/spot.py
--- a/acousticswarms-speech_amd/spot.py
+++ b/acousticswarms-speech_amd/spot.py
@@ -237,6 +237,11 @@
         native.check(native.lib().asw_spot_set_fused_mask(self._h, int(bool(on))))
         return self
 
+    def set_source_stack(self, on: bool = True):
+        self._need()
+        native.check(native.lib().asw_spot_set_source_stack(self._h, int(bool(on))))
+        return self
+
     def get_tap(self, name: str, shape=None):
         import torch
         n = c_size_t()
diff --git a/include/asw_hip.h b/include/asw_hip.h
--- a/include/asw_hip.h
+++ b/include/asw_hip.h
@@ -66,6 +66,8 @@
                      const float* window_embedding_host, float* out, void* stream);
 
 int asw_spot_set_fused_mask(asw_spot* m, int on);
+
+int asw_spot_set_source_stack(asw_spot* m, int on);
 
 int asw_spot_get_tap(asw_spot* m, const char* name, float* dst, size_t capacity, size_t* numel,
                      void* stream);
@@ -139,6 +141,10 @@
                                  const int32_t* mix_index, int N, int circular, const float* mean, const float* std,
                                  const float* w, const float* b, int C, float* x0, float* refn, long refn_stride,
                                  void* stream);
+
+int asw_shift_norm_src_multi(const float* mix, int M, int T, int T_pad, const int32_t* offsets,
+                             const int32_t* mix_index, int N, int circular, const float* mean, const float* std,
+                             void* src_hi, void* src_lo, float* refn, long refn_stride, void* stream);
 
 int asw_pad_preproc(const float* x, int B, int M, int t, int T_pad, const float* w,
                     const float* b, int C, float* x0, float* refn, long refn_stride,
@@ -217,8 +223,15 @@
   const float* glu_gamma;
   const float* glu_beta;
   float* glu_out;
+  const void* src_hi;
+  const void* src_lo;
+  const void* pre_hi;
+  const void* pre_lo;
+  int32_t pre_shift;
 } asw_resstack_args;
 int asw_resstack64_f16x3(const asw_resstack_args* args, void* stream);
+int asw_compose_source_weights(const float* wc, const float* wpre, const float* bpre, int M, int taps, float* comp,
+                               float* pre16);
 int asw_split_weights_f16(const float* w, size_t n, uint16_t* hi, uint16_t* lo, int32_t* w_shift);
 int asw_f16x3_overflow_count(int reset, uint32_t* count);
 int asw_convgemm_stats_tiles(int M_out, int N);
```

New measurement: 2408 candidates/s, median of 6. 2.4% higher.
